# alibaba/easydist

Measured on NVIDIA H100. Metric: train_step_throughput, higher is better.
Workload: dtype bf16

## Files before the change

### easydist_b200/_lib.py

```python
import ctypes
import os
from ctypes import (POINTER, c_char_p, c_float, c_int, c_int64, c_size_t, c_uint64, c_void_p)

from . import build as _build

EDB_OK, EDB_E_INVALID, EDB_E_UNSUPPORTED, EDB_E_CUDA, EDB_E_STATE = 0, 1, 2, 3, 4

DTYPE_CODES = {"float32": 0, "bfloat16": 1, "float16": 2, "float64": 3, "int32": 4, "int64": 5}
REDOP_CODES = {"sum": 0, "max": 1, "min": 2, "avg": 3}


class EdbError(RuntimeError):

    def __init__(self, code, msg):
        super().__init__(f"libedb error {code}: {msg}")
        self.code = code


class EdbUnsupported(EdbError):
    """The kernel does not cover this shape/layout; the dispatcher may route elsewhere."""


_I64P = POINTER(c_int64)
_IP = POINTER(c_int)

SIGNATURES = {
    "edb_version": (c_int, []),
    "edb_last_error": (c_char_p, []),
    "edb_init": (c_int, [c_int, c_int, c_int, c_size_t]),
    "edb_finalize": (c_int, []),
    "edb_is_initialized": (c_int, []),
    "edb_health": (c_int, []),
    "edb_heap_info": (c_int, [POINTER(c_void_p), POINTER(c_size_t), POINTER(c_size_t)]),
    "edb_ipc_export": (c_int, [c_void_p]),
    "edb_ipc_attach": (c_int, [c_int, c_void_p]),
    "edb_attach_local": (c_int, [c_int, c_void_p]),
    "edb_group_create": (c_int, [_IP, c_int, c_int, _IP]),
    "edb_group_info": (c_int, [c_int, _IP, _IP]),
    "edb_symm_alloc": (c_int, [c_size_t, c_size_t, POINTER(c_uint64)]),
    "edb_symm_mark": (c_int, [POINTER(c_uint64)]),
    "edb_symm_reset": (c_int, [c_uint64]),
    "edb_scatter": (c_int, [c_void_p, c_void_p, _I64P, c_int, c_int, c_int, c_int, c_int, _I64P,
                            c_void_p]),
    "edb_copy": (c_int, [c_void_p, c_void_p, c_size_t, c_void_p]),
    "edb_box_copy_local": (c_int, [c_void_p, _I64P, c_void_p, _I64P, _I64P, c_int, c_int,
                                   c_void_p]),
    "edb_all_gather": (c_int, [c_int, c_uint64, c_void_p, _I64P, c_int, c_int, c_int, c_void_p]),
    "edb_reduce_scatter": (c_int, [c_int, c_void_p, c_uint64, c_void_p, _I64P, c_int, c_int, c_int,
                                   c_int, c_float, c_int, c_void_p]),
    "edb_all_reduce": (c_int, [c_int, c_void_p, c_uint64, c_uint64, c_void_p, c_int64, c_int, c_int,
                               c_void_p]),
    "edb_all_to_all": (c_int, [c_int, c_void_p, c_uint64, c_void_p, _I64P, c_int, c_int, c_int,
                               c_int, c_void_p]),
    "edb_box_exchange": (c_int, [c_int, c_void_p, _I64P, c_uint64, c_void_p, _I64P, c_int, c_int,
                                 c_int, _IP, _I64P, _I64P, _I64P, _I64P, c_void_p]),
    "edb_halo_exchange": (c_int, [c_int, c_void_p, c_uint64, c_void_p, _I64P, c_int, c_int, c_int,
                                  c_int, c_void_p]),
    "edb_symm_guard": (c_int, [c_int, c_void_p]),
    "edb_gemm_bf16": (c_int, [c_void_p, c_void_p, c_void_p, c_void_p, c_int64, c_int64, c_int64,
                              c_int64, c_int64, c_int64, c_int, c_int, c_int, c_void_p]),
    "edb_ag_gemm_bf16": (c_int, [c_int, c_void_p, c_void_p, c_void_p, c_uint64, c_uint64, c_int64,
                                 c_int64, c_int64, c_int64, c_int64, c_void_p]),
    "edb_gemm_rs_bf16": (c_int, [c_int, c_void_p, c_uint64, c_void_p, c_void_p, c_int64, c_int64,
                                 c_int64, c_int64, c_int64, c_int, c_int, c_float, c_int,
                                 c_void_p]),
    "edb_gemm_rs_push_bf16": (c_int, [c_int, c_uint64, c_uint64, c_void_p, c_void_p, c_int64, c_int64,
                                      c_int64, c_int64, c_int64, c_int, c_int, c_void_p]),
    "edb_rs_finish": (c_int, [c_int, c_int, c_void_p, c_void_p, c_void_p, _I64P, c_float, c_int,
                              c_void_p]),
    "edb_epoch_barrier": (c_int, [c_int, c_void_p]),
    "edb_all_gather_push": (c_int, [c_int, c_uint64, c_void_p, _I64P, c_int, c_int, c_int, c_void_p]),
    "edb_all_to_all_push": (c_int, [c_int, c_uint64, c_void_p, _I64P, c_int, c_int, c_int, c_int,
                                    c_void_p]),
    "edb_reduce_scatter_push": (c_int, [c_int, c_void_p, c_uint64, c_void_p, _I64P, c_int, c_int,
                                        c_int, c_int, c_float, c_int, c_void_p]),
    "edb_all_reduce_push": (c_int, [c_int, c_uint64, c_uint64, c_void_p, c_int64, c_int, c_int,
                                    c_void_p]),
    "edb_ag_gemm_epoch_bf16": (c_int, [c_int, c_void_p, c_void_p, c_void_p, c_uint64, c_uint64,
                                       c_int64, c_int64, c_int64, c_int64, c_int64, c_void_p]),
    "edb_ag_prefetch": (c_int, [c_int, c_int, c_void_p, c_void_p, _I64P, _I64P, _I64P, c_void_p]),
    "edb_gemm_pf_bf16": (c_int, [c_void_p, c_void_p, c_void_p, c_void_p, c_int64, c_int64, c_int64,
                                 c_int64, c_int64, c_int64, c_int, c_int, c_int, c_int, c_void_p,
                                 c_void_p, _I64P, _I64P, _I64P, c_void_p]),
    "edb_gemm_epi_bf16": (c_int, [c_void_p, c_void_p, c_void_p, c_void_p, c_void_p, c_int64, c_int,
                                  c_int64, c_int64, c_int64, c_int64, c_int64, c_int64, c_int, c_int,
                                  c_int, c_int, c_void_p, c_void_p, _I64P, _I64P, _I64P, c_void_p]),
    "edb_gemm_push_bf16": (c_int, [c_int, c_uint64, c_void_p, c_void_p, c_int64, c_int64, c_int64,
                                   c_int64, c_int64, c_int, c_int, c_void_p]),
    "edb_rs_finish_local": (c_int, [c_int, c_int, c_void_p, c_void_p, _I64P, c_float, c_int,
                                    c_void_p]),
    "edb_layer_norm_fwd": (c_int, [c_void_p, c_void_p, c_void_p, c_void_p, c_void_p, c_void_p,
                                   c_int64, c_int64, c_float, c_int, c_void_p]),
    "edb_layer_norm_bwd": (c_int, [c_void_p, c_void_p, c_void_p, c_void_p, c_void_p, c_void_p,
                                   c_void_p, c_void_p, c_void_p, c_int64, c_int64, c_int, c_void_p]),
    "edb_layer_norm_bwd_add": (c_int, [c_void_p, c_void_p, c_void_p, c_void_p, c_void_p, c_void_p,
                                       c_void_p, c_void_p, c_void_p, c_void_p, c_int64, c_int64,
                                       c_int, c_void_p]),
    "edb_layer_norm_bwd_workspace": (c_int, [c_int64, POINTER(c_size_t)]),
    "edb_rms_norm_fwd": (c_int, [c_void_p, c_void_p, c_void_p, c_void_p, c_int64, c_int64, c_float,
                                 c_int, c_int, c_void_p]),
    "edb_rms_norm_bwd": (c_int, [c_void_p, c_void_p, c_void_p, c_void_p, c_void_p, c_void_p, c_void_p,
                                 c_void_p, c_int64, c_int64, c_int, c_int, c_void_p]),
    "edb_rms_norm_bwd_workspace": (c_int, [c_int64, POINTER(c_size_t)]),
    "edb_swiglu_fwd": (c_int, [c_void_p, c_void_p, c_void_p, c_int64, c_int, c_void_p]),
    "edb_rope": (c_int, [c_void_p, c_void_p, c_void_p, c_void_p, c_int64, c_int64, c_int64, c_int64,
                         _I64P, _I64P, c_int64, c_int, c_int, c_void_p]),
    "edb_swiglu_bwd": (c_int, [c_void_p, c_void_p, c_void_p, c_void_p, c_void_p, c_int64, c_int,
                               c_void_p]),
    "edb_embedding_fwd": (c_int, [c_void_p, c_void_p, c_void_p, c_void_p, c_void_p, c_int64, c_int64,
                                  c_int64, c_int64, c_int64, c_int, c_int, c_void_p]),
    "edb_embedding_bwd": (c_int, [c_void_p, c_int64, c_void_p, c_int64, c_void_p, c_void_p, c_int64,
                                  c_int64, c_int64, c_int64, c_int, c_int, c_int, c_void_p]),
    "edb_embedding_bwd_workspace": (c_int, [c_int64, c_int64, POINTER(c_size_t)]),
    "edb_colsum": (c_int,[c_void_p, c_void_p, c_void_p, c_int64, c_int64, c_int64, c_int, c_void_p]),
    "edb_colsum_workspace": (c_int, [c_int64, POINTER(c_size_t)]),
    "edb_cross_entropy_fwd": (c_int, [c_void_p, c_void_p, c_void_p, c_void_p, c_void_p, c_int64,
                                      c_void_p, c_int64, c_int64, c_int64, c_int, c_int, c_void_p]),
    "edb_cross_entropy_bwd": (c_int, [c_void_p, c_int64, c_void_p, c_int64, c_void_p, c_void_p,
                                      c_void_p, c_void_p, c_int64, c_int64, c_int64, c_int, c_int,
                                      c_void_p]),
    "edb_sgd_momentum": (c_int, [c_int, c_void_p, c_void_p, c_void_p, _I64P, c_float, c_float, c_float,
                                 c_int, c_void_p]),
    "edb_sgd_momentum_scaled": (c_int, [c_int, c_void_p, c_void_p, c_void_p, _I64P, c_float, c_float,
                                        c_float, c_void_p, c_int, c_void_p]),
    "edb_grad_sumsq": (c_int, [c_int, c_void_p, _I64P, c_void_p, c_void_p, c_int, c_int, c_void_p]),
    "edb_grad_sumsq_workspace": (c_int, [c_int, _I64P, c_int, POINTER(c_size_t)]),
    "edb_multi_scale_": (c_int, [c_int, c_void_p, _I64P, c_void_p, c_int, c_void_p]),
    "edb_set_option": (c_int, [c_char_p, c_int64]),
    "edb_get_option": (c_int, [c_char_p, POINTER(c_int64)]),
    "edb_launch_count": (c_uint64, []),
}

_lib = None


def lib_path():
    return _build.LIB_PATH


def load(build_if_missing=True):
    global _lib
    if _lib is not None:
        return _lib
    path = lib_path()
    if build_if_missing and _build._nvcc() is not None and _build.needs_build():
        _build.build()
    if not os.path.exists(path):
        raise EdbError(EDB_E_STATE,
                       f"{path} is missing and cannot be built here (no nvcc); run "
                       "`python -m easydist_b200.build` where nvcc is available")
    lib = ctypes.CDLL(path, mode=ctypes.RTLD_GLOBAL)
    for name, (restype, argtypes) in SIGNATURES.items():
        fn = getattr(lib, name)
        fn.restype = restype
        fn.argtypes = argtypes
    _lib = lib
    return lib


def check(rc):
    if rc == EDB_OK:
        return
    msg = load().edb_last_error().decode("utf-8", "replace")
    if rc == EDB_E_UNSUPPORTED:
        raise EdbUnsupported(rc, msg)
    raise EdbError(rc, msg)


def i64_array(values):
    values = [int(v) for v in values]
    return (c_int64 * max(1, len(values)))(*values)


def int_array(values):
    values = [int(v) for v in values]
    return (c_int * max(1, len(values)))(*values)
```

### easydist_b200/api.py

```python
import logging
from functools import update_wrapper
from typing import Any

import os

import torch
import torch.utils._pytree as pytree

from . import lowering
from . import reshard as _default_ops
from .compile import EDCompiledFunc, GraphIO, trace_train_step
from .device_mesh import get_device_mesh

logger = logging.getLogger(__name__)

DP_MODES = ("ddp", "zero2", "zero3")
PARALLEL_EXTENTION = {}


def register_parallel_method(parallel_mode: str, compiler_func=None):

    def wrapper(fn):
        PARALLEL_EXTENTION[parallel_mode] = fn
        return fn

    return wrapper if compiler_func is None else wrapper(compiler_func)


def _dp_group(mesh):
    if "dp" in mesh.dim_names:
        d = mesh.dim_names.index("dp")
    else:
        assert mesh.ndim == 1, "data-parallel modes need a mesh dim named 'dp'"
        d = 0
    return mesh.ranks_along(d), mesh.get_coordinate()[d]


def _flat_inputs(params, buffers, named_states, args, kwargs):
    return pytree.tree_flatten((params, buffers, named_states, args, kwargs))[0]


def _single_group(gm, ops, ranks):
    want = list(ranks)
    for nd in gm.graph.nodes:
        if nd.op == "call_function" and nd.target in ops.COMM_FUNCS:
            grp = nd.args[5] if nd.target is ops.all_to_all_start else \
                (nd.args[3] if nd.target is ops.reduce_scatter_start else nd.args[2])
            if list(grp) != want:
                return False
    return True


class _ParamIO:

    def __init__(self, param_ph, param_names):
        self.param_ph, self.param_names = list(param_ph), list(param_names)


def _finish(gm, params, buffers, named_states, args, kwargs, ops, native, io=None, ranks=None,
            fuse=True, fuse_rt=None, my_index=None, auto_io=None):
    flat = _flat_inputs(params, buffers, named_states, args, kwargs)
    lowering.propagate_local_meta(gm, flat)
    info = {}
    if io is None and os.environ.get("EDB_LOCALIZE_OPT", "1" if native else "0") == "1":
        info["localized_foreach"] = lowering.localize_foreach(gm, ops, my_rank=get_device_mesh().rank)
        lowering.propagate_local_meta(gm, flat)
    auto_pf = (native or fuse_rt is not None) and fuse and auto_io is not None and ranks is not None \
        and len(ranks) > 1 and os.environ.get("EDB_EPOCH", "1") == "1" \
        and os.environ.get("EDB_AG_PREFETCH", "1") == "1"
    bucket = os.environ.get("EDB_BUCKET_COMM", "0") == "1"
    if bucket and not auto_pf:
        info["bucketed"] = lowering.bucket_small_comm(gm, ops)
        lowering.propagate_local_meta(gm, flat)
    experimental = [k for k in ("EDB_OVERLAP", "EDB_RS_LANE", "EDB_GEMM_SIDE", "EDB_DEFER_RS")
                    if os.environ.get(k, "0") == "1"]
    if experimental and native:
        if os.environ.get("EDB_ALLOW_EXPERIMENTAL", "0") != "1":
            raise RuntimeError(
                f"{experimental}: experimental multi-stream switches are gated on GPUs (kernels that "
                "spin on peer / sibling CTAs are sized for an idle GPU and are not co-residency safe "
                "next to a second stream); set EDB_ALLOW_EXPERIMENTAL=1 to try them anyway")
        logger.warning("experimental switches %s enabled (EDB_ALLOW_EXPERIMENTAL=1): not "
                       "co-residency safe, not part of the measured configuration", experimental)
    overlap = os.environ.get("EDB_OVERLAP", "0") == "1" and io is not None and ranks is not None \
        and len(ranks) > 1
    if overlap:
        info["overlap"] = lowering.overlap_schedule(gm, io, ops)
    elif (native or fuse_rt is not None) and fuse and io is not None and ranks is not None \
            and len(ranks) > 1:
        if fuse_rt is None:
            from .runtime import get_runtime
            fuse_rt = get_runtime()
        rt = fuse_rt
        rehomed, nf = lowering.fuse_collective_gemms(gm, io, rt, ranks, ops, my_index=my_index)
        info["fused"] = nf
        name_of = {ph.name: io.param_names[i] for i, ph in enumerate(io.param_ph)}
        for ph_name, buf in rehomed.items():
            pname = name_of[ph_name]
            t = params[pname]
            home = buf.tensor(t.dtype, t.shape)
            home.copy_(t)
            params[pname] = home
        lowering.propagate_local_meta(gm, _flat_inputs(params, buffers, named_states, args,
                                                       kwargs))
    elif auto_pf:
        if fuse_rt is None:
            from .runtime import get_runtime
            fuse_rt = get_runtime()
        rt = fuse_rt
        rehomed, n_pf = lowering.prefetch_param_gathers(gm, auto_io, rt, ranks, ops, my_index=my_index)
        if rehomed:
            lowering.insert_epoch_barriers(gm, ranks, ops)
            name_of = dict(zip([ph.name for ph in auto_io.param_ph], auto_io.param_names))
            for ph_name, buf in rehomed.items():
                t = params[name_of[ph_name]]
                home = buf.tensor(t.dtype, t.shape)
                home.copy_(t)
                params[name_of[ph_name]] = home
            lowering.propagate_local_meta(gm, _flat_inputs(params, buffers, named_states, args, kwargs))
        info["fused"] = {"ag_mm": 0, "ag_pf": n_pf, "mm_rs": 0}
        if bucket:
            info["bucketed"] = lowering.bucket_small_comm(gm, ops)
            lowering.propagate_local_meta(gm, _flat_inputs(params, buffers, named_states, args, kwargs))
    info["comm_nodes"] = lowering.count_nodes(gm, ops)
    info["reinplaced_updates"] = lowering.reinplace_optimizer_updates(gm)
    if native:
        from .runtime import get_runtime
        push = ranks is not None and len(ranks) > 1 and os.environ.get("EDB_EPOCH", "1") == "1" \
            and os.environ.get("EDB_PUSH_COLL", "1") == "1" and hasattr(ops, "epoch_barrier") \
            and not overlap and _single_group(gm, ops, ranks)
        info["symm_bytes"] = lowering.assign_static_buffers(gm, get_runtime(), ops, push=push)
        if push and any(nd.kwargs.get("_push") for nd in gm.graph.nodes if nd.op == "call_function"):
            lowering.ensure_end_barrier(gm, ranks, ops)
            info["push_collectives"] = True
        counts = {}
        info["gemm_nodes"] = lowering.dispatch_compute(gm, counts)
        info["rms_norm_nodes"] = counts["rms_norm"]
        info["swiglu_nodes"] = counts["swiglu"]
        info["rope_nodes"] = counts["rope"]
        info["clip_nodes"] = counts["clip"]
        info["embed_nodes"] = counts["embed"]
        if ranks is not None and len(ranks) > 1 and (push or info.get("fused")):
            try:
                rep = lowering.verify_epoch_protocol(gm, ops, len(ranks))
            except Exception as e:
                rep = {"ok": None, "problems": [f"checker failed: {e!r}"]}
            info["epoch_check"] = {"ok": rep["ok"], "problems": rep["problems"][:5],
                                   "ranges": rep.get("ranges"), "items": rep.get("items")}
            if rep["problems"]:
                logger.error("epoch-protocol check: %s", rep["problems"][:5])
                if os.environ.get("EDB_VERIFY_STRICT", "0") == "1":
                    raise RuntimeError(f"epoch-protocol check failed: {rep['problems'][:5]}")
    gm.graph.lint()
    gm.recompile()
    return info


def _compile_dp(func, parallel_mode, tracing_mode, args, kwargs, *, ops=_default_ops,
                native=True, fuse=True, bucket_numel=None, fuse_rt=None):
    mode = parallel_mode.replace("b200_", "")
    assert mode in DP_MODES, parallel_mode
    ranks, my_index = _dp_group(get_device_mesh())
    n = len(ranks)
    if bucket_numel is None:
        bucket_numel = 65536 if native else 0

    def trace_and_rewrite(a, kw, warm_up=True):
        params, buffers, named_states, gm, module, opt = trace_train_step(func, a, kw, tracing_mode,
                                                                          warm_up=warm_up)
        io = GraphIO(gm, params, buffers, named_states)
        shard_info = {}
        if n > 1:
            if mode == "ddp":
                lowering.transform_ddp(gm, io, ranks, ops, bucket_numel=bucket_numel)
            else:
                _, shard_info = lowering.transform_fsdp(gm, io, ranks, my_index,
                                                        shard_param=(mode == "zero3"), ops=ops,
                                                        bucket_numel=bucket_numel)
        return params, buffers, named_states, gm, io, shard_info

    params, buffers, named_states, gm, io, shard_info = trace_and_rewrite(args, kwargs)
    with torch.no_grad():
        params = {k: v.detach() for k, v in params.items()}
        if shard_info:
            ph_names = {ph.name: i for i, ph in enumerate(io.param_ph)}
            for ph_name, idx in ph_names.items():
                if ph_name in shard_info:
                    name = io.param_names[idx]
                    params[name] = ops.scatter_wrapper(params[name].flatten(), n, 0, my_index)
            flat_states, spec = pytree.tree_flatten(named_states)
            for i, ph in enumerate(io.state_ph):
                if ph.name in shard_info and isinstance(flat_states[i], torch.Tensor):
                    flat_states[i] = ops.scatter_wrapper(flat_states[i].detach().flatten(), n, 0,
                                                         my_index)
            named_states = pytree.tree_unflatten(flat_states, spec)
    info = _finish(gm, params, buffers, named_states, args, kwargs, ops, native, io=io,
                   ranks=ranks, fuse=fuse, fuse_rt=fuse_rt, my_index=my_index)
    info.update(mode=mode, dp_size=n)
    if native and n > 1:
        from .runtime import get_runtime
        get_runtime().host_barrier()

    def mono_compiler(compiled, a, kw):
        _, _, _, gm2, io2, _ = trace_and_rewrite(a, kw, warm_up=False)
        p, b, st = compiled.get_state()
        _finish(gm2, p, b, st, a, kw, ops, native, io=io2, ranks=ranks, fuse=False)
        return gm2

    return EDCompiledFunc(gm, params, buffers, named_states, info=info, mono_compiler=mono_compiler)


def _lower_auto(gm, plan, state_io_map, params, buffers, named_states, args, kwargs, *, ops, native,
                planner, mesh, fuse_rt=None):
    n_p, n_b = len(params), len(buffers)
    flat_states, spec = pytree.tree_flatten(named_states)
    placeholders = [n for n in gm.graph.nodes if n.op == "placeholder"]
    param_ph = placeholders[:n_p]
    buffer_ph = placeholders[n_p:n_p + n_b]
    state_ph = placeholders[n_p + n_b:n_p + n_b + len(flat_states)]
    input_phs = placeholders[n_p + n_b + len(flat_states):]
    plan = lowering._normalise_plan(plan)
    lowering.sharding_transform(gm, plan, state_io_map, ops=ops, mesh=mesh, planner=planner)
    env = gm._edb_shard_env

    def shard_local(t, ph):
        strat = env.get(ph.name)
        if not isinstance(t, torch.Tensor) or strat is None:
            return t
        coord = mesh.get_coordinate()
        for mdim, s in enumerate(strat):
            if s.is_shard():
                t = ops.scatter_wrapper(t, mesh.size(mdim), s.dim, coord[mdim])
        return t

    with torch.no_grad():
        params = {k: shard_local(v.detach(), ph) for (k, v), ph in zip(params.items(), param_ph)}
        buffers = {k: shard_local(v.detach(), ph) for (k, v), ph in zip(buffers.items(),
                                                                       buffer_ph)}
        flat_states = [shard_local(s.detach() if isinstance(s, torch.Tensor) else s, ph)
                       for s, ph in zip(flat_states, state_ph)]
        named_states = pytree.tree_unflatten(flat_states, spec)

    def input_transform(a, kw):
        flat, spec_in = pytree.tree_flatten((a, kw))
        flat = [shard_local(x.detach() if isinstance(x, torch.Tensor) else x, ph)
                for x, ph in zip(flat, input_phs)]
        return pytree.tree_unflatten(flat, spec_in)

    largs, lkwargs = input_transform(args, kwargs)
    auto_io, ranks1d, my_index = None, None, None
    if mesh.ndim == 1:
        auto_io = _ParamIO(param_ph, list(params.keys()))
        ranks1d, my_index = mesh.ranks_along(0), mesh.get_coordinate()[0]
    info = _finish(gm, params, buffers, named_states, largs, lkwargs, ops, native, auto_io=auto_io,
                   ranks=ranks1d, my_index=my_index, fuse_rt=fuse_rt)
    info.update(mode="auto", mesh=mesh.shape)
    if native:
        from .runtime import get_runtime, is_initialized
        if is_initialized():
            get_runtime().host_barrier()
    return EDCompiledFunc(gm, params, buffers, named_states, input_transform=input_transform,
                          info=info)


def _compile_auto(func, tracing_mode, args, kwargs, *, plan=None, ops=_default_ops, native=True,
                  planner="GREEDY", bundle=None):
    mesh = get_device_mesh("spmd")
    if bundle is not None:
        return compile_from_bundle(bundle, args, kwargs, ops=ops, native=native, planner=planner)
    if plan is None:
        raise NotImplementedError(
            "parallel_mode='auto' needs a sharding plan: use easydist_b200.api.register() to run "
            "behind the reference's solver, or pass plan=<plan> / bundle=<recorded graph+plan>")
    params, buffers, named_states, gm, module, opt = trace_train_step(func, args, kwargs,
                                                                      tracing_mode)
    io = GraphIO(gm, params, buffers, named_states)
    return _lower_auto(gm, plan, io.state_io_map(), params, buffers, named_states, args, kwargs,
                       ops=ops, native=native, planner=planner, mesh=mesh)


def compile_from_bundle(bundle_text, args, kwargs, *, ops=_default_ops, native=True,
                        planner="GREEDY", fuse_rt=None):
    from . import graph_io
    from .compile import find_module_and_optimizer, warm_up_optimizer
    mesh = get_device_mesh("spmd")
    module, opt = find_module_and_optimizer(args, kwargs)
    device = next(module.parameters()).device
    gm, plan, state_io, _ = graph_io.load_bundle(bundle_text, device=device.type)
    params = dict(module.named_parameters())
    buffers = dict(module.named_buffers())
    named_states = warm_up_optimizer(module, opt)
    flat = [x.detach() if isinstance(x, torch.Tensor) else None
            for x in _flat_inputs(params, buffers, named_states, args, kwargs)]
    lowering.propagate_local_meta(gm, flat)
    class _Named:
        def __init__(self, name):
            self.name = name

    io_map = {_Named(a): _Named(b) for a, b in state_io}
    return _lower_auto(gm, plan, io_map, params, buffers, named_states, args, kwargs, ops=ops,
                       native=native, planner=planner, mesh=mesh, fuse_rt=fuse_rt)


LAST_AUTO_SOURCE = [None]


def _plan_cache_key(args, kwargs, mesh):
    import hashlib
    leaves, spec = pytree.tree_flatten((args, kwargs))
    parts = [repr(spec), repr(tuple(mesh.shape))]
    for x in leaves:
        if isinstance(x, torch.Tensor):
            parts.append(f"T{tuple(x.shape)}:{x.dtype}")
        elif isinstance(x, torch.nn.Module):
            parts.append(repr(x) + "|" + ",".join(f"{n}{tuple(p.shape)}{p.dtype}"
                                                  for n, p in x.named_parameters()))
        elif isinstance(x, torch.optim.Optimizer):
            parts.append(type(x).__qualname__ + repr([{k: v for k, v in g.items() if k != "params"}
                                                      for g in x.param_groups]))
        else:
            parts.append(repr(x))
    return hashlib.sha256("|".join(parts).encode("utf-8")).hexdigest()[:32]


def input_signature(args, kwargs):
    import hashlib
    leaves, spec = pytree.tree_flatten((args, kwargs))
    parts = [repr(spec)]
    for x in leaves:
        if isinstance(x, torch.Tensor):
            parts.append(f"T{tuple(x.shape)}:{x.dtype}")
        elif isinstance(x, (torch.nn.Module, torch.optim.Optimizer)):
            parts.append(f"{type(x).__qualname__}@{id(x):x}")
        else:
            parts.append(repr(x))
    return hashlib.sha256("|".join(parts).encode("utf-8")).hexdigest()


class CompiledFuncWrapper:

    def __init__(self, func, parallel_mode="auto", tracing_mode="fake", cuda_graph=True,
                 enable_mono_graph=False, compile_only=False, compile_kwargs=None):
        update_wrapper(self, func)
        self.original_func = func
        self.compiled_func = None
        self.parallel_mode = parallel_mode
        self.tracing_mode = tracing_mode
        self.enable_cuda_graph = cuda_graph
        self.enable_mono_graph = enable_mono_graph
        self.compile_only = compile_only
        self.compile_kwargs = compile_kwargs or {}
        self.all_input_signature = []
        self.graph_list = {}
        self.cuda_graph_space = {}
        self.graph_pool = None

    def _compile(self, args, kwargs):
        mode = self.parallel_mode
        if mode == "auto":
            return _compile_auto(self.original_func, self.tracing_mode, args, kwargs,
                                 **self.compile_kwargs)
        if mode in DP_MODES:
            return _compile_dp(self.original_func, mode, self.tracing_mode, args, kwargs,
                               **self.compile_kwargs)
        if mode in PARALLEL_EXTENTION:
            return PARALLEL_EXTENTION[mode](self.original_func, mode, self.tracing_mode, args,
                                            kwargs)
        raise NotImplementedError()

    def register_input_signature(self, *args, **kwargs):
        sig = input_signature(args, kwargs)
        if sig not in self.all_input_signature:
            self.all_input_signature.append(sig)
            if self.enable_cuda_graph:
                self.cuda_graph_space[sig] = {"cuda_graph": None, "cuda_graph_input": None,
                                              "cuda_graph_output": None}
        return sig

    def _run(self, sig, args, kwargs):
        if sig not in self.graph_list:
            if not self.enable_mono_graph:
                raise RuntimeError(
                    "Input mismatch. If you are sure that different inputs do not change the graph, "
                    "you can try turning on the enable_mono_graph option.")
            self.graph_list[sig] = self.compiled_func.compile_mono_graph(*args, **kwargs)
            logger.info(f"[Compile API] compile mono graph for {sig}")
        return self.compiled_func.run_with_graph(self.graph_list[sig], *args, **kwargs)

    def __call__(self, *args: Any, **kwargs: Any) -> Any:
        sig = self.register_input_signature(*args, **kwargs)
        if self.compiled_func is None:
            self.compiled_func = self._compile(args, kwargs)
            self.graph_list[sig] = self.compiled_func.graph
        if self.compile_only:
            return self.compiled_func
        if not self.enable_cuda_graph:
            return self._run(sig, args, kwargs)
        space = self.cuda_graph_space[sig]
        flat, spec = pytree.tree_flatten([args, kwargs])
        if space["cuda_graph"] is None:
            space["cuda_graph_input"] = [torch.empty_like(x).copy_(x) if isinstance(x, torch.Tensor)
                                         else x for x in flat]
            sargs, skwargs = pytree.tree_unflatten(space["cuda_graph_input"], spec)
            s = torch.cuda.Stream()
            s.wait_stream(torch.cuda.current_stream())
            with torch.cuda.stream(s):
                space["cuda_graph_output"] = self._run(sig, sargs, skwargs)
            torch.cuda.current_stream().wait_stream(s)
            torch.cuda.synchronize()
            space["cuda_graph"] = torch.cuda.CUDAGraph()
            with torch.cuda.graph(space["cuda_graph"], self.graph_pool):
                space["cuda_graph_output"] = self._run(sig, sargs, skwargs)
            if self.graph_pool is None:
                self.graph_pool = space["cuda_graph"].pool()
        else:
            for dst, src in zip(space["cuda_graph_input"], flat):
                if isinstance(dst, torch.Tensor):
                    dst.copy_(src, non_blocking=True)
        from .compile import _check_health
        _check_health()
        space["cuda_graph"].replay()
        return space["cuda_graph_output"]


def easydist_compile(func=None, parallel_mode="auto", tracing_mode="fake", cuda_graph=True,
                     enable_mono_graph=False, use_hint=False, liveness_only_input=False,
                     max_solver_time=float("inf"), compile_only=False, **compile_kwargs):
    if parallel_mode not in ("auto",) + DP_MODES and parallel_mode not in PARALLEL_EXTENTION:
        raise NotImplementedError(
            "please use [auto, ddp, zero2, zero3] for `parallel_mode` or register your parallel "
            "extention")

    def wrap(f):
        return CompiledFuncWrapper(f, parallel_mode, tracing_mode, cuda_graph, enable_mono_graph,
                                   compile_only, compile_kwargs)

    return wrap(func) if func else wrap


def register(reference_api=None, reference_compile_auto=None, **compile_kwargs):
    import easydist.torch.api as ref_api
    import easydist.torch.compile_auto as ref_auto
    reference_api = reference_api or ref_api
    reference_compile_auto = reference_compile_auto or ref_auto
# ... 75 lines not shown
```

### easydist_b200/build.py

```python
import hashlib
import os
import shutil
import subprocess
import sys
from concurrent.futures import ThreadPoolExecutor

HERE = os.path.dirname(os.path.abspath(__file__))
ROOT = os.path.dirname(HERE)
CSRC = os.path.join(HERE, "csrc")
INCLUDE = os.path.join(ROOT, "include")
LIB_PATH = os.path.join(HERE, "libedb.so")
BUILD_DIR = os.path.join(HERE, "csrc", "_build")

HEADERS = ["edb_internal.cuh", "edb_vec.cuh"]
SOURCES = ["edb_runtime.cu", "edb_reshard.cu", "edb_ll.cu", "edb_norm.cu", "edb_rms.cu", "edb_rope.cu", "edb_embed.cu", "edb_loss.cu", "edb_optim.cu", "edb_clip.cu", "edb_gemm.cu"]

ARCH = "arch=compute_90a,code=sm_90a"

NVCC_FLAGS = [
    "-std=c++17", "-O3", "-lineinfo",
    "-gencode", ARCH,
    "-Xcompiler", "-fPIC",
    "-I", INCLUDE, "-I", CSRC,
]


def _nvcc():
    cand = shutil.which("nvcc") or "/usr/local/cuda/bin/nvcc"
    return cand if os.path.exists(cand) else None


def _digest(paths):
    h = hashlib.sha256()
    for p in sorted(paths):
        with open(p, "rb") as f:
            h.update(p.encode())
            h.update(f.read())
    h.update(" ".join(NVCC_FLAGS).encode())
    return h.hexdigest()


def sources():
    return [os.path.join(CSRC, s) for s in SOURCES if os.path.exists(os.path.join(CSRC, s))]


def needs_build():
    stamp = os.path.join(BUILD_DIR, "stamp")
    if not os.path.exists(LIB_PATH) or not os.path.exists(stamp):
        return True
    deps = sources() + [os.path.join(CSRC, h) for h in HEADERS] + [os.path.join(INCLUDE, "edb.h")]
    with open(stamp) as f:
        return f.read().strip() != _digest(deps)


def build(force=False, verbose=False):
    if not force and not needs_build():
        return LIB_PATH
    import fcntl
    os.makedirs(BUILD_DIR, exist_ok=True)
    with open(os.path.join(BUILD_DIR, ".lock"), "w") as lock:
        fcntl.flock(lock, fcntl.LOCK_EX)
        try:
            if not force and not needs_build():
                return LIB_PATH
            return _build_locked(verbose)
        finally:
            fcntl.flock(lock, fcntl.LOCK_UN)


def _build_locked(verbose):
    import tempfile
    nvcc = _nvcc()
    if nvcc is None:
        raise RuntimeError("nvcc not found: cannot build libedb.so")
    srcs = sources()
    tmp = tempfile.mkdtemp(prefix="tmp_", dir=BUILD_DIR)
    objs = [os.path.join(tmp, os.path.basename(s)[:-3] + ".o") for s in srcs]

    def compile_one(args):
        src, obj = args
        cmd = [nvcc, *NVCC_FLAGS, "-c", src, "-o", obj]
        if verbose:
            cmd.insert(1, "-Xptxas=-v")
        r = subprocess.run(cmd, capture_output=True, text=True)
        if r.returncode != 0:
            raise RuntimeError(f"nvcc failed for {src}:\n{r.stdout}\n{r.stderr}")
        return r.stderr

    with ThreadPoolExecutor(max_workers=len(srcs)) as ex:
        logs = list(ex.map(compile_one, zip(srcs, objs)))
    if verbose:
        sys.stderr.write("\n".join(logs))
    tmp_lib = os.path.join(tmp, "libedb.so")
    cmd = [nvcc, "-shared", "-gencode", ARCH, "-o", tmp_lib, *objs]
    r = subprocess.run(cmd, capture_output=True, text=True)
    if r.returncode != 0:
        raise RuntimeError(f"link failed:\n{r.stdout}\n{r.stderr}")
    deps = srcs + [os.path.join(CSRC, h) for h in HEADERS] + [os.path.join(INCLUDE, "edb.h")]
    tmp_stamp = os.path.join(tmp, "stamp")
    with open(tmp_stamp, "w") as f:
        f.write(_digest(deps))
    os.replace(tmp_lib, LIB_PATH)
    os.replace(tmp_stamp, os.path.join(BUILD_DIR, "stamp"))
    shutil.rmtree(tmp, ignore_errors=True)
    return LIB_PATH


if __name__ == "__main__":
    print(build(force="--force" in sys.argv, verbose="-v" in sys.argv))
```

### easydist_b200/csrc/edb_gemm.cu

```cuda
#include <cuda.h>
#include <cuda_bf16.h>

#include "edb_internal.cuh"

namespace edb {

constexpr int BM = 128;
constexpr int BK = 64;
constexpr int MMA_K = 16;
constexpr int kConsumerThreads = 256;
constexpr int kGemmThreads = kConsumerThreads + 32;
constexpr int kSmemABytes = BM * BK * 2;

template <int BN> struct TileCfg {
  static constexpr int kSmemBBytes = BN * BK * 2;
  static constexpr int kStageBytes = kSmemABytes + kSmemBBytes;
  static constexpr int kStages = (BN == 256) ? 4 : 6;
  static constexpr int kEpiBufBytes = BM * 64 * 2;
  static constexpr int kEpiBufs = 2;
  static constexpr int kSmemBytes =
      kStages * kStageBytes + kEpiBufs * kEpiBufBytes + 1024  + 256 ;
};


__device__ __forceinline__ uint32_t smem_u32(const void* p) {
  return static_cast<uint32_t>(__cvta_generic_to_shared(p));
}
__device__ __forceinline__ void mbar_init(uint64_t* bar, uint32_t count) {
  asm volatile("mbarrier.init.shared::cta.b64 [%0], %1;" ::"r"(smem_u32(bar)), "r"(count));
}
__device__ __forceinline__ void mbar_expect_tx(uint64_t* bar, uint32_t bytes) {
  asm volatile("mbarrier.arrive.expect_tx.shared::cta.b64 _, [%0], %1;" ::"r"(smem_u32(bar)),
               "r"(bytes)
               : "memory");
}
__device__ __forceinline__ void mbar_arrive(uint64_t* bar) {
  asm volatile("mbarrier.arrive.shared::cta.b64 _, [%0];" ::"r"(smem_u32(bar)) : "memory");
}
__device__ __forceinline__ bool mbar_try_wait(uint32_t addr, uint32_t parity) {
  uint32_t ok;
  asm volatile(
      "{\n"
      ".reg .pred p;\n"
      "mbarrier.try_wait.parity.shared::cta.b64 p, [%1], %2;\n"
      "selp.u32 %0, 1, 0, p;\n"
      "}\n"
      : "=r"(ok)
      : "r"(addr), "r"(parity)
      : "memory");
  return ok != 0;
}
__device__ __forceinline__ void mbar_wait(uint64_t* bar, uint32_t parity) {
  const uint32_t addr = smem_u32(bar);
  if (mbar_try_wait(addr, parity)) return;
  const uint64_t t0 = globaltimer_ns();
  uint32_t spins = 0;
  while (!mbar_try_wait(addr, parity)) {
    if ((++spins & 0xfff) == 0 && globaltimer_ns() - t0 > 4000000000ull) {
      asm volatile("trap;");
    }
  }
}
__device__ __forceinline__ void fence_barrier_init() {
  asm volatile("fence.mbarrier_init.release.cluster;" ::: "memory");
}
__device__ __forceinline__ void fence_proxy_async() {
  asm volatile("fence.proxy.async.shared::cta;" ::: "memory");
}
__device__ __forceinline__ void tma_load_2d(const CUtensorMap* map, uint64_t* bar, void* smem,
                                            int c0, int c1) {
  asm volatile(
      "cp.async.bulk.tensor.2d.shared::cluster.global.mbarrier::complete_tx::bytes [%0], [%1, {%3, "
      "%4}], [%2];" ::"r"(smem_u32(smem)),
      "l"(map), "r"(smem_u32(bar)), "r"(c0), "r"(c1)
      : "memory");
}
__device__ __forceinline__ void tma_store_2d(const CUtensorMap* map, const void* smem, int c0,
                                             int c1) {
  asm volatile(
      "cp.async.bulk.tensor.2d.global.shared::cta.bulk_group [%0, {%2, %3}], [%1];" ::"l"(map),
      "r"(smem_u32(smem)), "r"(c0), "r"(c1)
      : "memory");
}
__device__ __forceinline__ void tma_store_commit() {
  asm volatile("cp.async.bulk.commit_group;" ::: "memory");
}
template <int N> __device__ __forceinline__ void tma_store_wait_read() {
  asm volatile("cp.async.bulk.wait_group.read %0;" ::"n"(N) : "memory");
}
__device__ __forceinline__ void tma_store_wait_all() {
  asm volatile("cp.async.bulk.wait_group 0;" ::: "memory");
}
__device__ __forceinline__ void epi_bar_sync() {
  asm volatile("bar.sync 1, %0;" ::"n"(kConsumerThreads) : "memory");
}
__device__ __forceinline__ void prefetch_tmap(const CUtensorMap* map) {
  asm volatile("prefetch.tensormap [%0];" ::"l"(map) : "memory");
}
__device__ __forceinline__ void wgmma_fence() {
  asm volatile("wgmma.fence.sync.aligned;" ::: "memory");
}
__device__ __forceinline__ void wgmma_commit() {
  asm volatile("wgmma.commit_group.sync.aligned;" ::: "memory");
}
template <int N> __device__ __forceinline__ void wgmma_wait() {
  asm volatile("wgmma.wait_group.sync.aligned %0;" ::"n"(N) : "memory");
}

template <int TA, int TB>
__device__ __forceinline__ void wgmma_m64n128k16(float* d, uint64_t desc_a, uint64_t desc_b,
                                                  uint32_t scale_d) {
  asm volatile(
      "{\n"
      ".reg .pred p;\n"
      "setp.ne.b32 p, %66, 0;\n"
      "wgmma.mma_async.sync.aligned.m64n128k16.f32.bf16.bf16 "
      "{"
      "%0, %1, %2, %3, %4, %5, %6, %7, %8, %9, %10, %11, %12, %13, %14, %15, "
      "%16, %17, %18, %19, %20, %21, %22, %23, %24, %25, %26, %27, %28, %29, %30, %31, "
      "%32, %33, %34, %35, %36, %37, %38, %39, %40, %41, %42, %43, %44, %45, %46, %47, "
      "%48, %49, %50, %51, %52, %53, %54, %55, %56, %57, %58, %59, %60, %61, %62, %63"
      "}, %64, %65, p, 1, 1, %67, %68;\n"
      "}\n"
      : "+f"(d[0]), "+f"(d[1]), "+f"(d[2]), "+f"(d[3]), "+f"(d[4]), "+f"(d[5]), "+f"(d[6]), "+f"(d[7]),
        "+f"(d[8]), "+f"(d[9]), "+f"(d[10]), "+f"(d[11]), "+f"(d[12]), "+f"(d[13]), "+f"(d[14]), "+f"(d[15]),
        "+f"(d[16]), "+f"(d[17]), "+f"(d[18]), "+f"(d[19]), "+f"(d[20]), "+f"(d[21]), "+f"(d[22]), "+f"(d[23]),
        "+f"(d[24]), "+f"(d[25]), "+f"(d[26]), "+f"(d[27]), "+f"(d[28]), "+f"(d[29]), "+f"(d[30]), "+f"(d[31]),
        "+f"(d[32]), "+f"(d[33]), "+f"(d[34]), "+f"(d[35]), "+f"(d[36]), "+f"(d[37]), "+f"(d[38]), "+f"(d[39]),
        "+f"(d[40]), "+f"(d[41]), "+f"(d[42]), "+f"(d[43]), "+f"(d[44]), "+f"(d[45]), "+f"(d[46]), "+f"(d[47]),
        "+f"(d[48]), "+f"(d[49]), "+f"(d[50]), "+f"(d[51]), "+f"(d[52]), "+f"(d[53]), "+f"(d[54]), "+f"(d[55]),
        "+f"(d[56]), "+f"(d[57]), "+f"(d[58]), "+f"(d[59]), "+f"(d[60]), "+f"(d[61]), "+f"(d[62]), "+f"(d[63])
      : "l"(desc_a), "l"(desc_b), "r"(scale_d), "n"(TA), "n"(TB));
}

template <int TA, int TB>
__device__ __forceinline__ void wgmma_m64n256k16(float* d, uint64_t desc_a, uint64_t desc_b,
                                                  uint32_t scale_d) {
  asm volatile(
      "{\n"
      ".reg .pred p;\n"
      "setp.ne.b32 p, %130, 0;\n"
      "wgmma.mma_async.sync.aligned.m64n256k16.f32.bf16.bf16 "
      "{"
      "%0, %1, %2, %3, %4, %5, %6, %7, %8, %9, %10, %11, %12, %13, %14, %15, "
      "%16, %17, %18, %19, %20, %21, %22, %23, %24, %25, %26, %27, %28, %29, %30, %31, "
      "%32, %33, %34, %35, %36, %37, %38, %39, %40, %41, %42, %43, %44, %45, %46, %47, "
      "%48, %49, %50, %51, %52, %53, %54, %55, %56, %57, %58, %59, %60, %61, %62, %63, "
      "%64, %65, %66, %67, %68, %69, %70, %71, %72, %73, %74, %75, %76, %77, %78, %79, "
      "%80, %81, %82, %83, %84, %85, %86, %87, %88, %89, %90, %91, %92, %93, %94, %95, "
      "%96, %97, %98, %99, %100, %101, %102, %103, %104, %105, %106, %107, %108, %109, %110, %111, "
      "%112, %113, %114, %115, %116, %117, %118, %119, %120, %121, %122, %123, %124, %125, %126, %127"
      "}, %128, %129, p, 1, 1, %131, %132;\n"
      "}\n"
      : "+f"(d[0]), "+f"(d[1]), "+f"(d[2]), "+f"(d[3]), "+f"(d[4]), "+f"(d[5]), "+f"(d[6]), "+f"(d[7]),
        "+f"(d[8]), "+f"(d[9]), "+f"(d[10]), "+f"(d[11]), "+f"(d[12]), "+f"(d[13]), "+f"(d[14]), "+f"(d[15]),
        "+f"(d[16]), "+f"(d[17]), "+f"(d[18]), "+f"(d[19]), "+f"(d[20]), "+f"(d[21]), "+f"(d[22]), "+f"(d[23]),
        "+f"(d[24]), "+f"(d[25]), "+f"(d[26]), "+f"(d[27]), "+f"(d[28]), "+f"(d[29]), "+f"(d[30]), "+f"(d[31]),
        "+f"(d[32]), "+f"(d[33]), "+f"(d[34]), "+f"(d[35]), "+f"(d[36]), "+f"(d[37]), "+f"(d[38]), "+f"(d[39]),
        "+f"(d[40]), "+f"(d[41]), "+f"(d[42]), "+f"(d[43]), "+f"(d[44]), "+f"(d[45]), "+f"(d[46]), "+f"(d[47]),
        "+f"(d[48]), "+f"(d[49]), "+f"(d[50]), "+f"(d[51]), "+f"(d[52]), "+f"(d[53]), "+f"(d[54]), "+f"(d[55]),
        "+f"(d[56]), "+f"(d[57]), "+f"(d[58]), "+f"(d[59]), "+f"(d[60]), "+f"(d[61]), "+f"(d[62]), "+f"(d[63]),
        "+f"(d[64]), "+f"(d[65]), "+f"(d[66]), "+f"(d[67]), "+f"(d[68]), "+f"(d[69]), "+f"(d[70]), "+f"(d[71]),
        "+f"(d[72]), "+f"(d[73]), "+f"(d[74]), "+f"(d[75]), "+f"(d[76]), "+f"(d[77]), "+f"(d[78]), "+f"(d[79]),
        "+f"(d[80]), "+f"(d[81]), "+f"(d[82]), "+f"(d[83]), "+f"(d[84]), "+f"(d[85]), "+f"(d[86]), "+f"(d[87]),
        "+f"(d[88]), "+f"(d[89]), "+f"(d[90]), "+f"(d[91]), "+f"(d[92]), "+f"(d[93]), "+f"(d[94]), "+f"(d[95]),
        "+f"(d[96]), "+f"(d[97]), "+f"(d[98]), "+f"(d[99]), "+f"(d[100]), "+f"(d[101]), "+f"(d[102]), "+f"(d[103]),
        "+f"(d[104]), "+f"(d[105]), "+f"(d[106]), "+f"(d[107]), "+f"(d[108]), "+f"(d[109]), "+f"(d[110]), "+f"(d[111]),
        "+f"(d[112]), "+f"(d[113]), "+f"(d[114]), "+f"(d[115]), "+f"(d[116]), "+f"(d[117]), "+f"(d[118]), "+f"(d[119]),
        "+f"(d[120]), "+f"(d[121]), "+f"(d[122]), "+f"(d[123]), "+f"(d[124]), "+f"(d[125]), "+f"(d[126]), "+f"(d[127])
      : "l"(desc_a), "l"(desc_b), "r"(scale_d), "n"(TA), "n"(TB));
}


__device__ __forceinline__ uint64_t make_smem_desc(uint32_t smem_addr, uint32_t lbo_bytes,
                                                   uint32_t sbo_bytes) {
  uint64_t d = 0;
  d |= (uint64_t)((smem_addr >> 4) & 0x3fff);
  d |= (uint64_t)((lbo_bytes >> 4) & 0x3fff) << 16;
  d |= (uint64_t)((sbo_bytes >> 4) & 0x3fff) << 32;
  d |= (uint64_t)1 << 62;
  return d;
}

struct GemmParams {
  __nv_bfloat16* C;
  const __nv_bfloat16* bias;
  int64_t ldc;
  int M, N, K;
  int m_tiles, n_tiles;
  int splits, kb_per_split;
  float* partial;
  int64_t ldp;
  int push_n, push_mtc, m_rot;
  int push_sync;
  const __nv_bfloat16* aux;
  int64_t ld_aux;
  int epi_op;
};
enum { EPI_NONE = 0, EPI_ADD = 1, EPI_GELU_BWD = 2 };

__device__ __forceinline__ float gelu_tanh_grad(float x) {
  const float kBeta = 0.7978845608028654f;
  const float kKappa = 0.044715f;
  const float x_sq = x * x;
  const float inner = kBeta * (x + kKappa * x_sq * x);
  const float au = fabsf(inner);
  float e;
  asm("ex2.approx.ftz.f32 %0, %1;" : "=f"(e) : "f"(-2.885390081777927f * au));
  float r;
  asm("rcp.approx.ftz.f32 %0, %1;" : "=f"(r) : "f"(1.0f + e));
  const float t = copysignf((1.0f - e) * r, inner);
  const float tanh_d = 4.0f * e * r * r;
  const float left = 0.5f * x, right = 1.0f + t;
  const float left_d = 0.5f * right;
  const float inner_d = kBeta * (1.0f + 3.0f * kKappa * x_sq);
  return left_d + left * tanh_d * inner_d;
}

enum { MODE_PLAIN = 0, MODE_AG = 1, MODE_RS = 2 };
constexpr int kMaxPfItems = 4;
constexpr int kPfSlots = 12, kPfDepth = 8;
constexpr int F_TILECNT = 96;

struct FusedArgs {
  FlagCtx f;
  int n_comm;
  const char* shard_src[kMaxGroup];
  char* full_dst;
  int64_t shard_bytes;
  int ag_rows;
  int ag_first_tile;
  char* recv_base;
  int64_t chunk_bytes;
  void* rs_dst;
  float rs_scale;
  int rs_out_dtype;
  int tiles_per_chunk;
  int rs_defer;
  uint64_t* rs_state;
  int epoch;
  int pf_ctas, pf_items, pf_n;
  const char* pf_heap[kMaxGroup];
  char* pf_local;
  uint64_t pf_src[kMaxPfItems], pf_dst[kMaxPfItems];
  int64_t pf_bytes[kMaxPfItems], pf_stride[kMaxPfItems];
  int64_t pf_sstride[kMaxPfItems];
  int pf_inplace[kMaxPfItems];
};
constexpr int F_PUSHED = F_CHUNK + 8;

struct CMaps {
  CUtensorMap m[kMaxGroup];
};

template <int MODE>
__device__ __forceinline__ void tile_coords(int t, const GemmParams& p, const FusedArgs& fa,
                                            int& m_blk, int& n_blk, int& chunk) {
  if (MODE == MODE_AG) {
    const int ni = t / p.m_tiles;
    n_blk = (fa.ag_first_tile + ni) % p.n_tiles;
    m_blk = t - ni * p.m_tiles;
    chunk = -1;
  } else if (MODE == MODE_RS) {
    const int mtc = p.m_tiles / fa.f.n;
    const int tpc = mtc * p.n_tiles;
    const int ci = t / tpc, w = t - ci * tpc;
    chunk = (fa.f.me + 1 + ci) % fa.f.n;
    m_blk = chunk * mtc + w % mtc;
    n_blk = w / mtc;
  } else {
    chunk = 0;
    m_blk = (t % p.m_tiles + p.m_rot) % p.m_tiles;
    n_blk = t / p.m_tiles;
  }
}

__device__ __forceinline__ void bulk_load(void* smem, const void* gsrc, uint32_t bytes,
                                          uint64_t* bar) {
  asm volatile(
      "cp.async.bulk.shared::cluster.global.mbarrier::complete_tx::bytes [%0], [%1], %2, [%3];" ::
          "r"(smem_u32(smem)),
      "l"(gsrc), "r"(bytes), "r"(smem_u32(bar))
      : "memory");
}
__device__ __forceinline__ void bulk_store(void* gdst, const void* smem, uint32_t bytes) {
  asm volatile("cp.async.bulk.global.shared::cta.bulk_group [%0], [%1], %2;" ::"l"(gdst),
               "r"(smem_u32(smem)), "r"(bytes)
               : "memory");
}
__device__ __forceinline__ void fence_proxy_async_all() {
  asm volatile("fence.proxy.async;" ::: "memory");
}
__device__ __forceinline__ void spin_wait_gpu(const uint64_t* flag, uint64_t target) {
  if (ld_acquire_gpu(flag) >= target) return;
  const uint64_t t0 = globaltimer_ns();
  uint32_t spins = 0;
  while (ld_acquire_gpu(flag) < target) {
    __nanosleep(32);
    if ((++spins & 0xfff) == 0 && globaltimer_ns() - t0 > 4000000000ull) asm volatile("trap;");
  }
}

__device__ __forceinline__ void pf_role(const FusedArgs& fa, uint8_t* smem, int idx, int nctas) {
  constexpr int S = kPfSlots, D = kPfDepth, SLOT = 16384;
  uint64_t* full = reinterpret_cast<uint64_t*>(smem + S * SLOT);
  if (threadIdx.x == 0) {
    for (int s = 0; s < S; ++s) mbar_init(&full[s], 1);
    fence_barrier_init();
  }
  __syncthreads();
  if (threadIdx.x != 0) return;
  uint32_t n_load = 0, n_store = 0;
  struct Cur { int it, k; int64_t blk; };
  auto advance = [&](Cur& c) {
    while (c.it < fa.pf_items) {
      const int64_t nblk = (fa.pf_bytes[c.it] + SLOT - 1) / SLOT;
      const int members = fa.pf_inplace[c.it] ? fa.pf_n - 1 : fa.pf_n;
      if (c.k < members && c.blk < nblk) return true;
      if (c.k < members) c.blk -= nblk;
      if (++c.k >= members) {
        c.k = 0;
        ++c.it;
      }
    }
    return false;
  };
  Cur ld = {0, 0, (int64_t)idx}, stc = {0, 0, (int64_t)idx};
  bool more = advance(ld);
  int inflight = 0;
  while (more || inflight > 0) {
    if (more && inflight < D) {
      const uint32_t slot = n_load % S;
      if (n_load >= (uint32_t)S) tma_store_wait_read<S - D - 1>();
      const int p = (fa.f.me + 1 + ld.k) % fa.pf_n;
      const int64_t off = ld.blk * SLOT;
      const int64_t left = fa.pf_bytes[ld.it] - off;
      const uint32_t bytes = (uint32_t)(left < SLOT ? left : SLOT);
      mbar_expect_tx(&full[slot], bytes);
      bulk_load(smem + slot * SLOT,
                fa.pf_heap[p] + fa.pf_src[ld.it] + (int64_t)p * fa.pf_sstride[ld.it] + off, bytes,
                &full[slot]);
      ++n_load;
      ++inflight;
      ld.blk += nctas;
      more = advance(ld);
      continue;
    }
    advance(stc);
    const uint32_t slot = n_store % S;
    mbar_wait(&full[slot], (n_store / S) & 1);
    const int p = (fa.f.me + 1 + stc.k) % fa.pf_n;
    const int64_t off = stc.blk * SLOT;
    const int64_t left = fa.pf_bytes[stc.it] - off;
    const uint32_t bytes = (uint32_t)(left < SLOT ? left : SLOT);
    bulk_store(fa.pf_local + fa.pf_dst[stc.it] + (int64_t)p * fa.pf_stride[stc.it] + off,
               smem + slot * SLOT, bytes);
    tma_store_commit();
    ++n_store;
    --inflight;
    stc.blk += nctas;
  }
  tma_store_wait_all();
}

__global__ void __launch_bounds__(32, 1) k_ag_prefetch(const __grid_constant__ FusedArgs fa) {
  extern __shared__ uint8_t pf_smem_raw[];
  uint8_t* smem = reinterpret_cast<uint8_t*>((reinterpret_cast<uintptr_t>(pf_smem_raw) + 1023) &
                                             ~static_cast<uintptr_t>(1023));
  pf_role(fa, smem, (int)blockIdx.x, (int)gridDim.x);
}

__device__ __forceinline__ void ag_comm_role_epoch(const FusedArgs& fa, uint8_t* smem, int comm_idx,
                                                   uint64_t q) {
  constexpr int S = 8, D = 5, SLOT = 16384, kLag = 2;
  uint64_t* full = reinterpret_cast<uint64_t*>(smem + S * SLOT);
  const FlagCtx& f = fa.f;
  if (threadIdx.x == 0) {
    for (int s = 0; s < S; ++s) mbar_init(&full[s], 1);
    fence_barrier_init();
  }
  __syncthreads();
  if (threadIdx.x != 0) return;
  const int64_t per = ((fa.shard_bytes + fa.n_comm - 1) / fa.n_comm + SLOT - 1) / SLOT * SLOT;
  const int64_t lo = (int64_t)comm_idx * per;
  const int64_t hi = lo + per < fa.shard_bytes ? lo + per : fa.shard_bytes;
  const int nblk = hi > lo ? (int)((hi - lo + SLOT - 1) / SLOT) : 0;
  const int total = nblk * f.n;
  auto announce = [&](int k) {
    const int c = (f.me + k) % f.n;
    const unsigned long long prev =
        atomicAdd(reinterpret_cast<unsigned long long*>(f.local + F_AGTILE + c), 1ULL);
    if (prev == (unsigned long long)fa.n_comm - 1) {
      f.local[F_AGTILE + c] = 0;
      __threadfence();
      st_release_gpu(f.local + F_AGCHUNK + c, q);
    }
  };
  if (nblk == 0) {
    for (int k = 0; k < f.n; ++k) announce(k);
  } else {
    uint32_t n_load = 0, n_store = 0;
    int next_announce = 0;
    for (int g = 0; g < total + D; ++g) {
      if (g < total) {
        const int k = g / nblk, i = g - k * nblk;
        const int c = (f.me + k) % f.n;
        const uint32_t slot = n_load % S;
        if (n_load >= (uint32_t)S) tma_store_wait_read<S - D - 1>();
        const int64_t left = hi - lo - (int64_t)i * SLOT;
        const uint32_t bytes = (uint32_t)(left < SLOT ? left : SLOT);
        mbar_expect_tx(&full[slot], bytes);
        bulk_load(smem + slot * SLOT, fa.shard_src[c] + lo + (int64_t)i * SLOT, bytes, &full[slot]);
        ++n_load;
      }
      if (g >= D) {
        const int j = g - D;
        const int k = j / nblk, i = j - k * nblk;
        const int c = (f.me + k) % f.n;
        const uint32_t slot = n_store % S;
        mbar_wait(&full[slot], (n_store / S) & 1);
        const int64_t left = hi - lo - (int64_t)i * SLOT;
        const uint32_t bytes = (uint32_t)(left < SLOT ? left : SLOT);
        bulk_store(fa.full_dst + (int64_t)c * fa.shard_bytes + lo + (int64_t)i * SLOT,
                   smem + slot * SLOT, bytes);
        tma_store_commit();
        ++n_store;
        if ((int)n_store - kLag >= (next_announce + 1) * nblk) {
          asm volatile("cp.async.bulk.wait_group %0;" ::"n"(kLag) : "memory");
          fence_proxy_async_all();
          __threadfence();
          while ((int)n_store - kLag >= (next_announce + 1) * nblk) announce(next_announce++);
        }
      }
    }
    tma_store_wait_all();
    fence_proxy_async_all();
    __threadfence();
    while (next_announce < f.n) announce(next_announce++);
  }
  const unsigned long long prev =
      atomicAdd(reinterpret_cast<unsigned long long*>(f.local + F_AGDONE), 1ULL);
  if (prev == (unsigned long long)fa.n_comm - 1) {
    f.local[F_AGDONE] = 0;
    while (ld_acquire_gpu(f.local + F_AGCNT) < (uint64_t)gridDim.x) __nanosleep(64);
    f.local[F_AGCNT] = 0;
    st_release_gpu(f.local + F_AGSEQ, q);
  }
}

__device__ __forceinline__ void ag_comm_role(const FusedArgs& fa, uint8_t* smem, int comm_idx,
                                             uint64_t q) {
  constexpr int S = 8, D = 4, SLOT = 16384;
  uint64_t* full = reinterpret_cast<uint64_t*>(smem + S * SLOT);
  const FlagCtx& f = fa.f;
  if (threadIdx.x == 0) {
    for (int s = 0; s < S; ++s) mbar_init(&full[s], 1);
    fence_barrier_init();
  }
  __syncthreads();
  if (threadIdx.x != 0) return;
  const int w_chunk = F_CHUNK, w_tile = F_TILECNT;
  if (comm_idx == 0) {
    __threadfence_system();
    for (int pidx = 0; pidx < f.n; ++pidx)
      if (pidx != f.me) st_release_sys(f.peer[pidx] + F_READY + f.me, q);
  }
  uint32_t n_load = 0, n_store = 0;
  const int64_t per = ((fa.shard_bytes + fa.n_comm - 1) / fa.n_comm + SLOT - 1) / SLOT * SLOT;
  const int64_t lo = (int64_t)comm_idx * per;
  const int64_t hi = lo + per < fa.shard_bytes ? lo + per : fa.shard_bytes;
  const int64_t nblk = hi > lo ? (hi - lo + SLOT - 1) / SLOT : 0;
  for (int k = 0; k < f.n; ++k) {
    const int c = (f.me + k) % f.n;
    if (c != f.me) spin_wait_sys(f.local + F_READY + c, q, f.timeout_ns, f.local + F_ERR);
    const char* src = fa.shard_src[c] + lo;
    char* dst = fa.full_dst + (int64_t)c * fa.shard_bytes + lo;
    for (int64_t i = 0; i < nblk + D; ++i) {
      if (i < nblk) {
        const uint32_t slot = n_load % S;
        if (n_load >= (uint32_t)S) tma_store_wait_read<S - D - 1>();
        const int64_t left = hi - lo - i * SLOT;
        const uint32_t bytes = (uint32_t)(left < SLOT ? left : SLOT);
        mbar_expect_tx(&full[slot], bytes);
        bulk_load(smem + slot * SLOT, src + i * SLOT, bytes, &full[slot]);
// ... 118 lines not shown

template <int BN, bool A_KMAJOR, bool B_KMAJOR, int MODE>
__global__ void __launch_bounds__(kGemmThreads, 1)
    k_gemm_bf16(const __grid_constant__ CUtensorMap tmap_a, const __grid_constant__ CUtensorMap tmap_b,
                const __grid_constant__ CUtensorMap tmap_c, const GemmParams p,
                const __grid_constant__ FusedArgs fa, const __grid_constant__ CMaps cm) {
  using Cfg = TileCfg<BN>;
  constexpr int kStages = Cfg::kStages;
  extern __shared__ uint8_t smem_raw[];
  uint8_t* smem = reinterpret_cast<uint8_t*>((reinterpret_cast<uintptr_t>(smem_raw) + 1023) &
                                             ~static_cast<uintptr_t>(1023));
  __shared__ uint64_t s_q;
  __shared__ int s_last;
  uint64_t q = 0;
  const int n_gemm_ctas = (MODE == MODE_AG) ? (int)gridDim.x - fa.n_comm
                                             : (MODE == MODE_PLAIN ? (int)gridDim.x - fa.pf_ctas : (int)gridDim.x);

  if (MODE == MODE_RS) {
    if (fa.rs_defer) {
      if (threadIdx.x == 0) s_q = ld_relaxed_gpu(fa.f.local + F_SEQ) + 1;
      if ((int)threadIdx.x < fa.f.n && (int)threadIdx.x != fa.f.me) {
        const uint64_t prev = ld_relaxed_gpu(fa.rs_state + 1);
        if (prev) spin_wait_sys(fa.f.local + F_DONE + threadIdx.x, prev, fa.f.timeout_ns, fa.f.local + F_ERR);
      }
      __syncthreads();
      q = s_q;
    } else {
      q = begin_op(fa.f, &s_q);
    }
  } else if (MODE == MODE_AG) {
    if (threadIdx.x == 0) {
      s_q = ld_relaxed_gpu(fa.f.local + (fa.epoch ? F_AGSEQ : F_SEQ)) + 1;
      atomicAdd(reinterpret_cast<unsigned long long*>(fa.f.local + (fa.epoch ? F_AGCNT : F_CNT_C)), 1ULL);
    }
    __syncthreads();
    q = s_q;
    if ((int)blockIdx.x < fa.n_comm) {
      if (fa.epoch) ag_comm_role_epoch(fa, smem, (int)blockIdx.x, q);
      else ag_comm_role(fa, smem, (int)blockIdx.x, q);
      return;
    }
  }
  if (MODE == MODE_PLAIN && fa.pf_ctas > 0 && (int)blockIdx.x < fa.pf_ctas) {
    pf_role(fa, smem, (int)blockIdx.x, fa.pf_ctas);
    return;
  }
  const int cta = (MODE == MODE_AG) ? (int)blockIdx.x - fa.n_comm
                                    : (MODE == MODE_PLAIN ? (int)blockIdx.x - fa.pf_ctas : (int)blockIdx.x);

  uint8_t* smem_a = smem;
  uint8_t* smem_b = smem + kStages * kSmemABytes;
  uint8_t* smem_epi = smem + kStages * Cfg::kStageBytes;
  uint64_t* bars = reinterpret_cast<uint64_t*>(smem_epi + Cfg::kEpiBufs * Cfg::kEpiBufBytes);
  uint64_t* full_bar = bars;
  uint64_t* empty_bar = bars + kStages;

  const int warp = threadIdx.x >> 5;
  const int lane = threadIdx.x & 31;
  const int k_blocks = (p.K + BK - 1) / BK;
  const int num_tiles = p.m_tiles * p.n_tiles;
  const int num_units = (MODE == MODE_PLAIN) ? num_tiles * p.splits : num_tiles;

  if (threadIdx.x == 0) {
    for (int s = 0; s < kStages; ++s) {
      mbar_init(&full_bar[s], 1);
      mbar_init(&empty_bar[s], 2);
    }
    fence_barrier_init();
  }
  __syncthreads();

  if (warp == kConsumerThreads / 32) {
    if (lane == 0) {
      prefetch_tmap(&tmap_a);
      prefetch_tmap(&tmap_b);
      int stage = 0;
      uint32_t phase = 0;
      int ready_chunk = -1;
      for (int u = cta; u < num_units; u += n_gemm_ctas) {
        const int t = (MODE == MODE_PLAIN) ? u % num_tiles : u;
        int kb0 = 0, kb1 = k_blocks;
        if (MODE == MODE_PLAIN && p.splits > 1) {
          kb0 = (u / num_tiles) * p.kb_per_split;
          kb1 = kb0 + p.kb_per_split < k_blocks ? kb0 + p.kb_per_split : k_blocks;
        }
        int m_blk, n_blk, chunk;
        tile_coords<MODE>(t, p, fa, m_blk, n_blk, chunk);
        const CUtensorMap* bmap = &tmap_b;
        int b_row = n_blk * BN;
        if (MODE == MODE_AG) {
          const int c_lo = (n_blk * BN) / fa.ag_rows, c_hi = (n_blk * BN + BN - 1) / fa.ag_rows;
          if (c_lo == fa.f.me && c_hi == fa.f.me) {
            bmap = &cm.m[0];
            b_row = n_blk * BN - fa.f.me * fa.ag_rows;
          } else if (n_blk != ready_chunk) {
            for (int c = c_lo; c <= c_hi; ++c)
              spin_wait_gpu(fa.f.local + (fa.epoch ? F_AGCHUNK : F_CHUNK) + c, q);
            fence_proxy_async_all();
            ready_chunk = n_blk;
          }
        }
        for (int kb = kb0; kb < kb1; ++kb) {
          mbar_wait(&empty_bar[stage], phase ^ 1);
          uint8_t* sa = smem_a + stage * kSmemABytes;
          uint8_t* sb = smem_b + stage * Cfg::kSmemBBytes;
          mbar_expect_tx(&full_bar[stage], Cfg::kStageBytes);
          if (A_KMAJOR) {
            tma_load_2d(&tmap_a, &full_bar[stage], sa, kb * BK, m_blk * BM);
          } else {
#pragma unroll
            for (int h = 0; h < BM / 64; ++h)
              tma_load_2d(&tmap_a, &full_bar[stage], sa + h * (64 * BK * 2), m_blk * BM + h * 64,
                          kb * BK);
          }
          if (B_KMAJOR) {
            tma_load_2d(bmap, &full_bar[stage], sb, kb * BK, b_row);
          } else {
#pragma unroll
            for (int h = 0; h < BN / 64; ++h)
              tma_load_2d(bmap, &full_bar[stage], sb + h * (64 * BK * 2), b_row + h * 64, kb * BK);
          }
          if (++stage == kStages) {
            stage = 0;
            phase ^= 1;
          }
        }
      }
    }
  } else {
    const int wg = warp >> 2;
    const int tid = threadIdx.x & 127;
    const int frag_row = 16 * (tid >> 5) + ((tid & 31) >> 2);
    const int frag_col = 2 * (tid & 3);
    const int row0 = wg * 64 + frag_row;
    const bool issuer = (threadIdx.x == 0);
    if (issuer) prefetch_tmap(&tmap_c);
    float acc[BN / 2];
    int stage = 0;
    uint32_t phase = 0;
    int ebuf = 0;
    for (int u = cta; u < num_units; u += n_gemm_ctas) {
      const int t = (MODE == MODE_PLAIN) ? u % num_tiles : u;
      int kb0 = 0, kb1 = k_blocks;
      if (MODE == MODE_PLAIN && p.splits > 1) {
        kb0 = (u / num_tiles) * p.kb_per_split;
        kb1 = kb0 + p.kb_per_split < k_blocks ? kb0 + p.kb_per_split : k_blocks;
      }
      int m_blk, n_blk, chunk;
      tile_coords<MODE>(t, p, fa, m_blk, n_blk, chunk);

      int prev = -1;
      for (int kb = kb0; kb < kb1; ++kb) {
        mbar_wait(&full_bar[stage], phase);
        wgmma_fence();
        mma_k_block<BN, A_KMAJOR, B_KMAJOR>(acc, smem_u32(smem_a + stage * kSmemABytes) + wg * (64 * BK * 2),
                                            smem_u32(smem_b + stage * Cfg::kSmemBBytes), kb == kb0);
        wgmma_commit();
        wgmma_wait<1>();
        if (prev >= 0 && tid == 0) mbar_arrive(&empty_bar[prev]);
        prev = stage;
        if (++stage == kStages) {
          stage = 0;
          phase ^= 1;
        }
      }
      wgmma_wait<0>();
      if (prev >= 0 && tid == 0) mbar_arrive(&empty_bar[prev]);

      if (MODE == MODE_PLAIN && p.splits > 1) {
#pragma unroll
        for (int h = 0; h < 2; ++h) {
          const int64_t r = (int64_t)m_blk * BM + row0 + 8 * h;
          if (r >= p.M) continue;
          float* prow = p.partial + ((int64_t)(u / num_tiles) * p.M + r) * p.ldp;
#pragma unroll
          for (int j = 0; j < BN / 8; ++j) {
            const int col = n_blk * BN + 8 * j + frag_col;
            if (col < p.ldp)
              *reinterpret_cast<float2*>(prow + col) = make_float2(acc[4 * j + 2 * h], acc[4 * j + 2 * h + 1]);
          }
        }
        continue;
      }
      const CUtensorMap* cmap = &tmap_c;
      int c_row = m_blk * BM;
      if (MODE == MODE_RS) {
        cmap = &cm.m[chunk];
        c_row = (m_blk - chunk * (p.m_tiles / fa.f.n)) * BM;
      }
      if (MODE == MODE_PLAIN && p.push_n > 0) {
        const int owner = m_blk / p.push_mtc;
        cmap = &cm.m[owner];
        c_row = (m_blk - owner * p.push_mtc) * BM;
      }
      const bool has_aux = (MODE == MODE_PLAIN && p.epi_op != EPI_NONE);
#pragma unroll
      for (int c0 = 0; c0 < BN; c0 += 64) {
        float* v = acc + c0 / 2;
        if (p.bias != nullptr) {
#pragma unroll
          for (int j = 0; j < 8; ++j) {
            const int col = n_blk * BN + c0 + 8 * j + frag_col;
            if (col < p.N) {
              const float2 f = __bfloat1622float2(*reinterpret_cast<const __nv_bfloat162*>(p.bias + col));
#pragma unroll
              for (int h = 0; h < 2; ++h) {
                v[4 * j + 2 * h] += f.x;
                v[4 * j + 2 * h + 1] += f.y;
              }
            }
          }
        }
        if (has_aux) {
#pragma unroll
          for (int h = 0; h < 2; ++h) {
            const int64_t r = (int64_t)m_blk * BM + row0 + 8 * h;
            const __nv_bfloat16* arow = p.aux + r * p.ld_aux;
#pragma unroll
            for (int j = 0; j < 8; ++j) {
              const int col = n_blk * BN + c0 + 8 * j + frag_col;
              float2 f = make_float2(0.f, 0.f);
              if (r < p.M && col < p.N)
                f = __bfloat1622float2(*reinterpret_cast<const __nv_bfloat162*>(arow + col));
              float x0 = v[4 * j + 2 * h], x1 = v[4 * j + 2 * h + 1];
              if (p.epi_op == EPI_ADD) {
                x0 += f.x;
                x1 += f.y;
              } else {
                x0 = __bfloat162float(__float2bfloat16_rn(x0)) * gelu_tanh_grad(f.x);
                x1 = __bfloat162float(__float2bfloat16_rn(x1)) * gelu_tanh_grad(f.y);
              }
              v[4 * j + 2 * h] = x0;
              v[4 * j + 2 * h + 1] = x1;
            }
          }
        }
        if (issuer) tma_store_wait_read<Cfg::kEpiBufs - 1>();
        epi_bar_sync();
        uint8_t* buf = smem_epi + ebuf * Cfg::kEpiBufBytes;
#pragma unroll
        for (int h = 0; h < 2; ++h) {
          const int row = row0 + 8 * h;
          uint8_t* rowp = buf + row * 128 + frag_col * 2;
#pragma unroll
          for (int j = 0; j < 8; ++j) {
            __nv_bfloat162 o = __floats2bfloat162_rn(v[4 * j + 2 * h], v[4 * j + 2 * h + 1]);
            *reinterpret_cast<__nv_bfloat162*>(rowp + ((j ^ (row & 7)) << 4)) = o;
          }
        }
        fence_proxy_async();
        epi_bar_sync();
        if (issuer) {
          tma_store_2d(cmap, buf, n_blk * BN + c0, c_row);
          tma_store_commit();
        }
        ebuf ^= 1;
      }
      if (MODE == MODE_RS && issuer) {
        tma_store_wait_all();
        fence_proxy_async_all();
        __threadfence_system();
        const unsigned long long prev_cnt = atomicAdd(
            reinterpret_cast<unsigned long long*>(fa.f.local + F_TILECNT + chunk), 1ULL);
        if (prev_cnt == (unsigned long long)fa.tiles_per_chunk - 1) {
          fa.f.local[F_TILECNT + chunk] = 0;
          __threadfence_system();
          st_release_sys(fa.f.peer[chunk] + (fa.rs_defer ? F_PUSHED : F_CHUNK) + fa.f.me, q);
        }
      }
    }
    if (issuer) {
      if (MODE == MODE_PLAIN && p.push_n > 0 && p.push_sync == 0) {
        tma_store_wait_read<0>();
      } else {
        tma_store_wait_all();
        if (MODE == MODE_PLAIN && p.push_n > 0 && p.push_sync >= 2) {
          fence_proxy_async_all();
          __threadfence_system();
        }
      }
    }
  }

  if (MODE == MODE_RS) {
    __syncthreads();
    if (fa.rs_defer) {
      if (blockIdx.x == 0 && threadIdx.x == 0) fa.rs_state[0] = q;
    } else {
      if (threadIdx.x < fa.f.n)
        spin_wait_sys(fa.f.local + F_CHUNK + threadIdx.x, q, fa.f.timeout_ns, fa.f.local + F_ERR);
      __syncthreads();
      const uint64_t tid = (uint64_t)blockIdx.x * blockDim.x + threadIdx.x;
      const uint64_t nthr = (uint64_t)gridDim.x * blockDim.x;
      if (fa.rs_out_dtype == EDB_F32) rs_tail_reduce<float>(fa, tid, nthr);
      else rs_tail_reduce<__nv_bfloat16>(fa, tid, nthr);
    }
    finish_op(fa.f, q, &s_last, gridDim.x);
  }
}

constexpr int kGemm2Threads = 384;
constexpr int kGemm2EpiBufBytes = 64 * 64 * 2;

template <int R> __device__ __forceinline__ void setmaxnreg_dec() {
  asm volatile("setmaxnreg.dec.sync.aligned.u32 %0;" ::"n"(R));
}
template <int R> __device__ __forceinline__ void setmaxnreg_inc() {
  asm volatile("setmaxnreg.inc.sync.aligned.u32 %0;" ::"n"(R));
}
__device__ __forceinline__ void wg_bar_sync(int wg) {
  if (wg == 0) asm volatile("bar.sync 1, 128;" ::: "memory");
  else asm volatile("bar.sync 2, 128;" ::: "memory");
}
__device__ __forceinline__ bool mbar_wait_ok(uint64_t* bar, uint32_t parity) {
  const uint32_t addr = smem_u32(bar);
  if (mbar_try_wait(addr, parity)) return true;
  const uint64_t t0 = globaltimer_ns();
  uint32_t spins = 0;
  while (!mbar_try_wait(addr, parity)) {
    if ((++spins & 0xfff) == 0 && globaltimer_ns() - t0 > 4000000000ull) return false;
  }
  return true;
}

template <bool A_KMAJOR, bool B_KMAJOR>
__global__ void __launch_bounds__(kGemm2Threads, 1)
    k_gemm2_bf16(const __grid_constant__ CUtensorMap tmap_a, const __grid_constant__ CUtensorMap tmap_b,
                 const __grid_constant__ CUtensorMap tmap_c, const GemmParams p) {
  constexpr int BN = 256;
  using Cfg = TileCfg<BN>;
  constexpr int kStages = Cfg::kStages;
  extern __shared__ uint8_t smem_raw[];
  uint8_t* smem = reinterpret_cast<uint8_t*>((reinterpret_cast<uintptr_t>(smem_raw) + 1023) &
                                             ~static_cast<uintptr_t>(1023));
  uint8_t* smem_a = smem;
  uint8_t* smem_b = smem + kStages * kSmemABytes;
  uint8_t* smem_epi = smem + kStages * Cfg::kStageBytes;
  uint64_t* full_bar = reinterpret_cast<uint64_t*>(smem_epi + Cfg::kEpiBufs * Cfg::kEpiBufBytes);
  uint64_t* empty_bar = full_bar + kStages;

  const int wgi = threadIdx.x >> 7;
  const int k_blocks = (p.K + BK - 1) / BK;
  const int mt = p.m_tiles;
  const int num_units = mt * p.n_tiles;

  if (threadIdx.x == 0) {
    for (int s = 0; s < kStages; ++s) {
      mbar_init(&full_bar[s], 1);
      mbar_init(&empty_bar[s], 2);
    }
    fence_barrier_init();
  }
  __syncthreads();

  bool ok = true;
  if (wgi == 0) {
    setmaxnreg_dec<40>();
    if (threadIdx.x == 0) {
      prefetch_tmap(&tmap_a);
      prefetch_tmap(&tmap_b);
      int stage = 0;
      uint32_t phase = 0;
      for (int u = blockIdx.x; ok && u < num_units; u += gridDim.x) {
        const int m_blk = u % mt, n_blk = u / mt;
        for (int kb = 0; kb < k_blocks; ++kb) {
          if (!(ok = mbar_wait_ok(&empty_bar[stage], phase ^ 1))) break;
          uint8_t* sa = smem_a + stage * kSmemABytes;
          uint8_t* sb = smem_b + stage * Cfg::kSmemBBytes;
          mbar_expect_tx(&full_bar[stage], Cfg::kStageBytes);
          if (A_KMAJOR) {
            tma_load_2d(&tmap_a, &full_bar[stage], sa, kb * BK, m_blk * BM);
          } else {
#pragma unroll
            for (int h = 0; h < BM / 64; ++h)
              tma_load_2d(&tmap_a, &full_bar[stage], sa + h * (64 * BK * 2), m_blk * BM + h * 64,
                          kb * BK);
          }
          if (B_KMAJOR) {
            tma_load_2d(&tmap_b, &full_bar[stage], sb, kb * BK, n_blk * BN);
          } else {
#pragma unroll
            for (int h = 0; h < BN / 64; ++h)
              tma_load_2d(&tmap_b, &full_bar[stage], sb + h * (64 * BK * 2), n_blk * BN + h * 64,
                          kb * BK);
          }
          if (++stage == kStages) {
            stage = 0;
            phase ^= 1;
          }
        }
      }
    }
  } else {
    setmaxnreg_inc<232>();
    const int wg = wgi - 1;
    const int tid = threadIdx.x & 127;
    const int frag_row = 16 * (tid >> 5) + ((tid & 31) >> 2);
    const int frag_col = 2 * (tid & 3);
    const int row0 = wg * 64 + frag_row;
    const bool issuer = (tid == 0);
    uint8_t* epi = smem_epi + wg * (2 * kGemm2EpiBufBytes);
    if (issuer) prefetch_tmap(&tmap_c);
    const int epi_op = p.epi_op;
    float acc[BN / 2];
    int stage = 0;
    uint32_t phase = 0;
    int ebuf = 0;
    for (int u = blockIdx.x; u < num_units; u += gridDim.x) {
      const int m_blk = u % mt, n_blk = u / mt;
      int prev = -1;
      for (int kb = 0; kb < k_blocks; ++kb) {
        if (!(ok = mbar_wait_ok(&full_bar[stage], phase))) break;
        wgmma_fence();
        mma_k_block<BN, A_KMAJOR, B_KMAJOR>(acc, smem_u32(smem_a + stage * kSmemABytes) + wg * (64 * BK * 2),
                                            smem_u32(smem_b + stage * Cfg::kSmemBBytes), kb == 0);
        wgmma_commit();
        wgmma_wait<1>();
        if (prev >= 0 && tid == 0) mbar_arrive(&empty_bar[prev]);
        prev = stage;
        if (++stage == kStages) {
          stage = 0;
          phase ^= 1;
        }
      }
      wgmma_wait<0>();
      if (!ok) break;
      if (prev >= 0 && tid == 0) mbar_arrive(&empty_bar[prev]);

#pragma unroll
      for (int c0 = 0; c0 < BN; c0 += 64) {
        float* v = acc + c0 / 2;
        if (p.bias != nullptr) {
#pragma unroll
          for (int j = 0; j < 8; ++j) {
            const int col = n_blk * BN + c0 + 8 * j + frag_col;
            if (col < p.N) {
              const float2 f = __bfloat1622float2(*reinterpret_cast<const __nv_bfloat162*>(p.bias + col));
#pragma unroll
              for (int h = 0; h < 2; ++h) {
                v[4 * j + 2 * h] += f.x;
                v[4 * j + 2 * h + 1] += f.y;
              }
            }
          }
        }
        if (epi_op != EPI_NONE) {
#pragma unroll
          for (int h = 0; h < 2; ++h) {
            const int64_t r = (int64_t)m_blk * BM + row0 + 8 * h;
            const __nv_bfloat16* arow = p.aux + r * p.ld_aux;
#pragma unroll
            for (int j = 0; j < 8; ++j) {
              const int col = n_blk * BN + c0 + 8 * j + frag_col;
              float2 f = make_float2(0.f, 0.f);
              if (r < p.M && col < p.N)
                f = __bfloat1622float2(*reinterpret_cast<const __nv_bfloat162*>(arow + col));
              float x0 = v[4 * j + 2 * h], x1 = v[4 * j + 2 * h + 1];
              if (epi_op == EPI_ADD) {
                x0 += f.x;
                x1 += f.y;
              } else {
                x0 = __bfloat162float(__float2bfloat16_rn(x0)) * gelu_tanh_grad(f.x);
                x1 = __bfloat162float(__float2bfloat16_rn(x1)) * gelu_tanh_grad(f.y);
              }
              v[4 * j + 2 * h] = x0;
              v[4 * j + 2 * h + 1] = x1;
            }
          }
        }
        if (issuer) tma_store_wait_read<1>();
        wg_bar_sync(wg);
        uint8_t* buf = epi + ebuf * kGemm2EpiBufBytes;
#pragma unroll
        for (int h = 0; h < 2; ++h) {
          const int row = frag_row + 8 * h;
          uint8_t* rowp = buf + row * 128 + frag_col * 2;
#pragma unroll
          for (int j = 0; j < 8; ++j) {
            __nv_bfloat162 o = __floats2bfloat162_rn(v[4 * j + 2 * h], v[4 * j + 2 * h + 1]);
            *reinterpret_cast<__nv_bfloat162*>(rowp + ((j ^ (row & 7)) << 4)) = o;
          }
        }
        fence_proxy_async();
        wg_bar_sync(wg);
        if (issuer) {
          tma_store_2d(&tmap_c, buf, n_blk * BN + c0, m_blk * BM + wg * 64);
          tma_store_commit();
        }
        ebuf ^= 1;
      }
    }
    if (issuer) tma_store_wait_all();
  }
  if (!ok) asm volatile("trap;");
}

constexpr int kRsMaxItems = 160;
constexpr int kRsFinishThreads = 256;
constexpr int64_t kRsFinishChunkVecs = 4096;

struct RsFinishItem {
  const char* recv;
  void* dst;
  int64_t chunk_bytes;
  uint64_t* state;
};
struct RsFinishDesc {
  FlagCtx f;
  int local_only;
  int n_items;
  float scale;
  int out_dtype;
  int first_unit[kRsMaxItems + 1];
  RsFinishItem it[kRsMaxItems];
};

template <int NSRC>
__global__ void __launch_bounds__(kRsFinishThreads, 4)
    k_rs_finish(const __grid_constant__ RsFinishDesc d) {
  __shared__ uint64_t s_q;
  __shared__ unsigned long long s_need;
  __shared__ int s_last;
  if (threadIdx.x == 0) {
    s_q = ld_relaxed_gpu(d.f.local + F_SEQ) + 1;
    s_need = 0;
  }
  __syncthreads();
  if (!d.local_only) {
    unsigned long long need = 0;
    for (int i = threadIdx.x; i < d.n_items; i += blockDim.x) {
      const unsigned long long e = ld_relaxed_gpu(d.it[i].state);
      need = e > need ? e : need;
    }
    if (need) atomicMax(&s_need, need);
    __syncthreads();
    if ((int)threadIdx.x < d.f.n)
      spin_wait_sys(d.f.local + F_PUSHED + threadIdx.x, s_need, d.f.timeout_ns, d.f.local + F_ERR);
    __syncthreads();
  }
  const uint64_t q = s_q;
  const int total_units = d.first_unit[d.n_items];
  const int n = NSRC > 0 ? NSRC : d.f.n;
  constexpr int MAXS = NSRC > 0 ? NSRC : kMaxGroup;
  constexpr int U = NSRC > 0 ? (8 / NSRC > 0 ? 8 / NSRC : 1) : 1;
  for (int u = blockIdx.x; u < total_units; u += gridDim.x) {
    int lo = 0, hi = d.n_items;
    while (hi - lo > 1) {
      const int mid = (lo + hi) >> 1;
      if (d.first_unit[mid] <= u) lo = mid;
      else hi = mid;
    }
    const char* recv = d.it[lo].recv;
    void* dst = d.it[lo].dst;
    const int64_t chunk_bytes = d.it[lo].chunk_bytes;
    const int64_t nvec = chunk_bytes / 16;
    const int64_t v0 = (int64_t)(u - d.first_unit[lo]) * kRsFinishChunkVecs;
    const int64_t v1 = v0 + kRsFinishChunkVecs < nvec ? v0 + kRsFinishChunkVecs : nvec;
    for (int64_t i0 = v0 + threadIdx.x; i0 < v1; i0 += U * kRsFinishThreads) {
      uint4 raw[U][MAXS];
#pragma unroll
      for (int uu = 0; uu < U; ++uu) {
        const int64_t i = i0 + uu * kRsFinishThreads;
        if (i < v1) {
#pragma unroll
          for (int sidx = 0; sidx < MAXS; ++sidx)
            if (sidx < n)
              raw[uu][sidx] = __ldcs(reinterpret_cast<const uint4*>(recv + (int64_t)sidx * chunk_bytes + i * 16));
        }
      }
#pragma unroll
      for (int uu = 0; uu < U; ++uu) {
        const int64_t i = i0 + uu * kRsFinishThreads;
        if (i >= v1) break;
        float acc[8];
#pragma unroll
        for (int sidx = 0; sidx < MAXS; ++sidx) {
          if (sidx < n) {
            const __nv_bfloat162* h = reinterpret_cast<const __nv_bfloat162*>(&raw[uu][sidx]);
#pragma unroll
            for (int e = 0; e < 4; ++e) {
              const float2 v = __bfloat1622float2(h[e]);
              if (sidx == 0) {
                acc[2 * e] = v.x;
                acc[2 * e + 1] = v.y;
              } else {
                acc[2 * e] += v.x;
                acc[2 * e + 1] += v.y;
              }
            }
          }
        }
#pragma unroll
        for (int e = 0; e < 8; ++e) acc[e] *= d.scale;
        if (d.out_dtype == EDB_F32) rs_store<float>(static_cast<float*>(dst), i, acc);
        else rs_store<__nv_bfloat16>(static_cast<__nv_bfloat16*>(dst), i, acc);
      }
    }
  }
  if (d.local_only) return;
  if (blockIdx.x == 0)
    for (int i = threadIdx.x; i < d.n_items; i += blockDim.x) d.it[i].state[1] = q;
  finish_op(d.f, q, &s_last, gridDim.x);
}

struct PushDst {
  int n;
  int64_t rows_per, row_rot;
  __nv_bfloat16* base[kMaxGroup];
};

__global__ void __launch_bounds__(256)
    k_splitk_reduce(__nv_bfloat16* __restrict__ C, int64_t ldc, const float* __restrict__ partial,
// ... 721 lines not shown
```

### easydist_b200/lowering.py

```python
import operator
import os
from typing import Dict

import torch
import torch.utils._pytree as pytree
from torch.fx.node import Node

from . import metair as M
from . import planners
from . import reshard as _default_ops
from .device_mesh import get_device_mesh

aten = torch.ops.aten

CREATE_ATEN_OP = [
    aten.empty.memory_format, aten.zeros.default, aten.ones.default, aten.scalar_tensor.default,
    aten.arange.default, aten.arange.start, aten.full.default,
]



def local_shape(global_shape, mesh, placements):
    shape = list(global_shape)
    coord = mesh.get_coordinate()
# ... 1458 lines not shown
               for nd in skip1 + skip2 for a in pytree.tree_flatten((nd.args, nd.kwargs))[0]):
            continue
        if mul.kwargs or set(add1.kwargs) - {"alpha"} or set(add2.kwargs) - {"alpha"}:
            continue
        if mul.users or add1.users or add2.users or len(mul.args) != 2:
            continue
        bufs, mu = mul.args
        if not isinstance(mu, (int, float)) or len(add1.args) != 2 or len(add2.args) != 2:
            continue
        if list(add1.args[0]) != list(bufs) or list(add2.args[1]) != list(bufs):
            continue
        grads, params = add1.args[1], add2.args[0]
        if not (len(grads) == len(bufs) == len(params)):
            continue
        if set(params) & set(bufs) or set(grads) & set(bufs) or set(grads) & set(params):
            continue
        ga, nlr = add1.kwargs.get("alpha", 1), add2.kwargs.get("alpha", 1)
        if not isinstance(ga, (int, float)) or not isinstance(nlr, (int, float)):
            continue
        with graph.inserting_before(add2):
            graph.call_function(optim.sgd_momentum_, (list(params), list(grads), list(bufs), mu, ga, nlr))
        for d in (add2, add1, mul):
            graph.erase_node(d)
        n += 1
    if n:
        gm.recompile()
    return n


_ALIAS_OPS = (aten.t.default, aten.view.default, aten._unsafe_view.default, aten.transpose.int,
              aten.permute.default, aten.alias.default, aten.detach.default, aten.slice.Tensor,
              aten.select.int, aten.flatten.using_ints, aten.reshape.default, aten.expand.default,
              aten.unsqueeze.default, aten.squeeze.dim, aten.as_strided.default)
_VIEW_ONLY = (aten.t.default, aten.view.default, aten._unsafe_view.default, aten.transpose.int,
              aten.permute.default, aten.alias.default, aten.detach.default, aten.unsqueeze.default,
              aten.squeeze.dim)


def _memory_readers(x, through=_ALIAS_OPS):
    root = x
    while _call(root, *through):
        root = root.args[0]
    readers, frontier, seen = [], [root], {root}
    while frontier:
        nd = frontier.pop()
        for u in nd.users:
            if u in seen:
                continue
            seen.add(u)
            if _call(u, *through) and u.args[0] is nd:
                frontier.append(u)
            else:
                readers.append(u)
    return readers


def _fold_clip_scale(gm, clamp):
    from . import clip, optim
    graph = gm.graph
    dt = _val(clamp).dtype if _val(clamp) is not None else None
    muls = [u for u in clamp.users if _call(u, aten.mul_.Tensor) and len(u.args) == 2
            and u.args[1] is clamp and u.args[0] is not clamp and not u.kwargs
            and _val(u.args[0]) is not None and _val(u.args[0]).dtype == dt]
    if not muls or len({m.args[0] for m in muls}) != len(muls):
        return 0
    pos = {nd: i for i, nd in enumerate(graph.nodes)}
    muls.sort(key=lambda m: pos[m])
    group = set(muls)
    users = {u for m in muls for u in m.users}
    sgd = next(iter(users)) if len(users) == 1 else None
    if _call(sgd, optim.sgd_momentum_) and "grad_scale" not in sgd.kwargs \
            and all(len(m.users) == 1 for m in muls) and set(sgd.args[1]) == group \
            and len(sgd.args[1]) == len(muls) \
            and not any(pos[r] > pos[m] and r not in group
                        for m in muls for r in _memory_readers(m.args[0])):
        args = list(sgd.args)
        args[1] = [m.args[0] for m in args[1]]
        sgd.args = tuple(args)
        sgd.kwargs = dict(sgd.kwargs, grad_scale=clamp)
        for m in muls:
            graph.erase_node(m)
        return len(muls)
    first = pos[muls[0]]
    for m in muls:
        if any(first < pos[r] < pos[m] and r not in group for r in _memory_readers(m.args[0])):
            return 0
    with graph.inserting_before(muls[0]):
        graph.call_function(clip.scale_, ([m.args[0] for m in muls], clamp))
    for m in muls:
        m.replace_all_uses_with(m.args[0])
        graph.erase_node(m)
    return len(muls)


def fuse_grad_clip(gm):
    from . import clip
    graph = gm.graph
    n_norm = n_scale = 0
    for ch in _match_clip(gm):
        norms, stack = ch["norms"], ch["stack"]
        dts = {_val(nd).dtype for nd in norms if _val(nd) is not None}
        if len(dts) != 1 or any(_val(nd.args[0]) is None or _val(nd.args[0]).dtype not in dts
                                for nd in norms):
            continue
        with graph.inserting_before(stack):
            gn = graph.call_function(clip.grad_norms, ([nd.args[0] for nd in norms],))
        gn.meta = dict(stack.meta)
        stack.replace_all_uses_with(gn)
        graph.erase_node(stack)
        for nd in norms:
            graph.erase_node(nd)
        n_norm += len(norms)
    for total in [nd for nd in graph.nodes if _is_norm2(nd)]:
        coef = _clip_coef(total)
        if coef is not None:
            n_scale += _fold_clip_scale(gm, coef[0])
    if n_norm or n_scale:
        graph.lint()
        gm.recompile()
    return n_norm, n_scale


def _embedding_pair(add):
    pair = _bin(add, aten.add.Tensor)
    if pair is None or not all(_call(e, aten.embedding.default) and _only_user(e) is add for e in pair):
        return None
    vals = [(_val(e.args[0]), _val(e.args[1])) for e in pair]
    if _val(add) is None or any(w is None or i is None for w, i in vals) or vals[0][0].dtype != vals[1][0].dtype:
        return None
    for tok, pos in ((0, 1), (1, 0)):
        (w, idx), (p, ps) = vals[tok], vals[pos]
        if ps.dim() == 1 and idx.dim() >= 1 and idx.shape[-1] == ps.shape[0] \
                and tuple(_val(add).shape) == tuple(idx.shape) + (w.shape[1],):
            return pair[tok], pair[pos]
    return None


def _tied_lm_gradient(bwd):
    from . import gemm
    add = _only_user(bwd)
    x = _other(_bin(add, aten.add.Tensor), bwd)
    root = x
    while _call(root, *_VIEW_ONLY):
        root = root.args[0]
    if not _call(root, gemm.mm) or root.kwargs.get("_side") or _memory_readers(x) != [add]:
        return None
    xv, bv, av = _val(x), _val(bwd), _val(add)
    if xv is None or bv is None or av is None or xv.dim() != 2 or xv.stride(1) != 1 \
            or tuple(xv.shape) != tuple(bv.shape) or tuple(av.shape) != tuple(xv.shape) \
            or not xv.dtype == bv.dtype == av.dtype:
        return None
    return add, x


def fuse_embedding(gm):
    from . import embed
    graph = gm.graph
    n_fwd = n_bwd = 0
    for nd in [nd for nd in graph.nodes if _call(nd, aten.add.Tensor)]:
        m = _embedding_pair(nd)
        if m is not None:
            tok, pos = m
            with graph.inserting_before(nd):
                new = graph.call_function(embed.embedding_fwd, (*tok.args[:2], *pos.args[:2]))
            new.meta = dict(nd.meta)
            nd.replace_all_uses_with(new)
            _erase_dead(graph, [nd, tok, pos])
            n_fwd += 1
    for nd in list(graph.nodes):
        if _call(nd, aten.embedding.default):
            nd.target, nd.args, nd.kwargs = embed.embedding_fwd, tuple(nd.args[:2]), {}
            n_fwd += 1
        elif _call(nd, aten.embedding_dense_backward.default) and len(nd.args) == 5 \
                and not nd.kwargs and nd.args[4] is False:
            dy, idx, V, pad, _ = nd.args
            tied = _tied_lm_gradient(nd)
            if tied is not None:
                add, x = tied
                with graph.inserting_before(add):
                    new = graph.call_function(embed.embedding_bwd_acc_, (x, dy, idx, pad))
                new.meta = dict(add.meta)
                add.replace_all_uses_with(new)
                _erase_dead(graph, [add, nd])
            else:
                nd.target, nd.args = embed.embedding_bwd, (dy, idx, V, pad)
            n_bwd += 1
    if n_fwd or n_bwd:
        graph.lint()
        gm.recompile()
    return n_fwd, n_bwd


def parallel_wgrad_gemms(gm):
    from . import gemm
    graph = gm.graph
    nodes = list(graph.nodes)
    order = {n: i for i, n in enumerate(nodes)}
    moved = 0
    for node in reversed(nodes):
        if node.op != "call_function" or node.target is not gemm.mm or node.kwargs:
            continue
        consumers = _memory_readers(node, _VIEW_ONLY)
        if not consumers:
            continue
        first = min(consumers, key=lambda u: order[u])
        between = nodes[order[node] + 1:order[first]]
        if not any(b.op == "call_function" and b.target in (gemm.mm, gemm.addmm)
                   and not b.kwargs.get("_side") for b in between):
            continue
        node.kwargs = {"_side": 1}
        with graph.inserting_before(first):
            graph.call_function(gemm.join, args=(node,))
        moved += 1
    if moved:
        graph.lint()
        gm.recompile()
    return moved


def fuse_gemm_epilogues(gm):
    from . import gemm, norm
    graph = gm.graph
    n = 0
    bf16 = torch.bfloat16

    def gemm_behind(nd):
        chain = []
        while _call(nd, aten.view.default, aten._unsafe_view.default) and len(nd.users) == 1:
            chain.append(nd)
            nd = nd.args[0]
        if _call(nd, gemm.mm, gemm.addmm) and len(nd.users) == 1 and not nd.kwargs.get("_side"):
            return nd, chain
        return None, chain

    def fuse(node, g, chain, target, operand, *extra):
        gv, ov, nv = _val(g), _val(operand), _val(node)
        with graph.inserting_before(g):
            op2d = operand if ov.dim() == 2 else graph.call_function(
                aten.view.default, args=(operand, list(gv.shape)))
            a, b = g.args[-2:]
            fused = graph.call_function(target, args=(a, b, op2d, *extra),
                                        kwargs={k: v for k, v in g.kwargs.items() if k == "_pf"})
            fused.meta = dict(g.meta)
            out = fused
            if nv.dim() != 2:
                out = graph.call_function(aten.view.default, args=(fused, list(nv.shape)))
                out.meta = dict(node.meta)
        node.replace_all_uses_with(out)
        _erase_dead(graph, [node, *chain, g])

    for node in list(graph.nodes):
        if node.op != "call_function":
            continue
        if node.target == aten.add.Tensor and len(node.args) == 2 and not node.kwargs:
            for gi, oi in ((1, 0), (0, 1)):
                g, chain = gemm_behind(node.args[gi])
                other = node.args[oi]
                gv, ov, nv = _val(g), _val(other), _val(node)
                if gv is None or ov is None or nv is None:
                    continue
                if ov.dtype != bf16 or gv.dtype != bf16 or gv.shape[1] % 8 or \
                        tuple(ov.shape) != tuple(nv.shape) or ov.numel() != gv.numel():
                    continue
                if not ov.is_contiguous():
                    continue
                order = {nd: i for i, nd in enumerate(graph.nodes)}
                if order[other] > order[g]:
                    continue
                fuse(node, g, chain, gemm.mm_add, other, g.args[0] if g.target is gemm.addmm else None)
                n += 1
                break
        elif node.target == aten.gelu_backward.default and node.kwargs.get("approximate") == "tanh":
            g, chain = gemm_behind(node.args[0])
            pre = node.args[1]
            gv, pv, nv = _val(g), _val(pre), _val(node)
            if g is None or g.target is not gemm.mm or gv is None or pv is None or nv is None:
                continue
            if pv.dtype != bf16 or gv.dtype != bf16 or gv.shape[1] % 8 or pv.numel() != gv.numel() \
                    or not pv.is_contiguous():
                continue
            order = {nd: i for i, nd in enumerate(graph.nodes)}
            if order[pre] > order[g]:
                continue
            fuse(node, g, chain, gemm.mm_gelu_bwd, pre)
            n += 1
    n += _fold_accumulation(graph, norm.native_layer_norm_backward)
    if n:
        graph.lint()
        gm.recompile()
    return n


def _reshape_views_of(node):
    frontier = [node]
    while frontier:
        nd = frontier.pop()
        for u in nd.users:
            if _call(u, *_ALIAS_OPS) and u.args[0] is nd:
                if u.target in (aten.view.default, aten._unsafe_view.default):
                    u.target = aten.reshape.default
                frontier.append(u)


def dispatch_compute(gm, counts=None):
    from . import gemm, norm
    native_ln = os.environ.get("EDB_NATIVE_LN", "1") == "1"
    counts = {} if counts is None else counts
    n = 0
    if os.environ.get("EDB_NATIVE_CE", "1") == "1":
        n += fuse_cross_entropy(gm)
    if os.environ.get("EDB_NATIVE_OPT", "1") == "1":
        n += fuse_optimizer_updates(gm)
    counts["rms_norm"] = fuse_rms_norm(gm) if os.environ.get("EDB_NATIVE_RMS", "1") == "1" else (0, 0)
    counts["swiglu"] = fuse_swiglu(gm) if os.environ.get("EDB_NATIVE_SWIGLU", "1") == "1" else (0, 0)
    counts["rope"] = fuse_rope(gm) if os.environ.get("EDB_NATIVE_ROPE", "1") == "1" else (0, 0)
    counts["clip"] = fuse_grad_clip(gm) if os.environ.get("EDB_NATIVE_CLIP", "1") == "1" else (0, 0)
    n += sum(counts["rms_norm"]) + sum(counts["swiglu"]) + sum(counts["rope"]) + sum(counts["clip"])
    for node in gm.graph.nodes:
        if node.op != "call_function":
            continue
        val = _val(node)
        if native_ln and node.target == aten.native_layer_norm.default:
            node.target = norm.native_layer_norm
            n += 1
        elif native_ln and node.target == aten.native_layer_norm_backward.default:
            node.target = norm.native_layer_norm_backward
            n += 1
        elif native_ln and node.target == aten.sum.dim_IntList:
            node.target = norm.sum_dim_intlist
            n += 1
        elif val is None or val.dtype != torch.bfloat16:
            continue
        elif node.target == aten.mm.default:
            node.target = gemm.mm
            if "edb_pf" in node.meta:
                node.kwargs = {"_pf": node.meta["edb_pf"]}
            if val.dim() == 2 and val.shape[1] % 8:
                _reshape_views_of(node)
            n += 1
        elif node.target == aten.addmm.default and not node.kwargs:
            node.target = gemm.addmm
            if "edb_pf" in node.meta:
                node.kwargs = {"_pf": node.meta["edb_pf"]}
            n += 1
    gm.recompile()
    counts["embed"] = fuse_embedding(gm) if os.environ.get("EDB_NATIVE_EMBED", "1") == "1" else (0, 0)
    n += sum(counts["embed"])
    if os.environ.get("EDB_GEMM_SIDE", "0") == "1":
        n += parallel_wgrad_gemms(gm)
    if os.environ.get("EDB_FUSE_EPILOGUE", "1") == "1":
        n += fuse_gemm_epilogues(gm)
    return n


def prefetch_param_gathers(gm, io, rt, ranks, ops=_default_ops, my_index=None):
    import os
    from collections import deque
    graph = gm.graph
    n = len(ranks)
    order = {nd: i for i, nd in enumerate(graph.nodes)}
    uses = {}
    dim1_ok = os.environ.get("EDB_AG_PREFETCH_DIM1", "1") == "1"
    for ag_s in [x for x in graph.nodes if x.op == "call_function" and x.target is ops.all_gather_start]:
        ph, n_t = ag_s.args[0], 0
        while isinstance(ph, Node) and ph.op == "call_function" and ph.target == aten.t.default and \
                isinstance(ph.args[0], Node):
            ph, n_t = ph.args[0], n_t + 1
        transposed = bool(n_t % 2)
        if not (isinstance(ph, Node) and ph.op == "placeholder" and ph in io.param_ph):
            continue
        val = ph.meta.get("val")
        if not isinstance(val, torch.Tensor) or (val.numel() * val.element_size()) % 16 or val.numel() == 0:
            continue
        if n_t and val.dim() != 2:
            continue
        d = ag_s.args[1]
        if not isinstance(d, int):
            continue
        d = d + val.dim() if d < 0 else d
        wdim = 1 - d if transposed else d
        if wdim == 1 and not (val.dim() == 2 and dim1_ok):
            continue
        if wdim not in (0, 1) or list(ag_s.args[2]) != list(ranks) \
                or ag_s.kwargs or len(ag_s.users) != 1 or not val.is_contiguous():
            continue
        ag_e = next(iter(ag_s.users))
        if ag_e.target is not ops.all_gather_end:
            continue
        uses.setdefault(ph, []).append((ag_s, ag_e, transposed, wdim))
    uses = {ph: lst for ph, lst in uses.items() if len({u[3] for u in lst}) == 1}
    if not uses:
        return {}, 0
    rehomed, bufs = {}, {}
    for ph in uses:
        nbytes = _nbytes(ph.meta["val"])
        full = rt.alloc(nbytes * n, align=1024)
        if my_index is None:
            shard = rt.alloc(nbytes, align=1024)
        else:
            shard = full.sub(int(my_index) * nbytes, nbytes)
        rehomed[ph.name] = shard
        bufs[ph] = (shard, full, nbytes)
    gathered_nodes = {}
    for ph, lst in uses.items():
        shard, full, nbytes = bufs[ph]
        pv = ph.meta["val"]
        for ag_s, ag_e, transposed, wdim in lst:
            with graph.inserting_before(ag_s):
                g = graph.call_function(ops.gathered, args=(ph, list(ranks)),
                                        kwargs={"_buf": (shard.offset, full.offset)})
                res = g
                if wdim == 1:
                    r_, c_ = pv.shape
                    res = graph.call_function(aten.view.default, args=(g, [n, r_, c_]))
                    res = graph.call_function(aten.permute.default, args=(res, [1, 0, 2]))
                    res = graph.call_function(aten.reshape.default, args=(res, [r_, n * c_]))
                elif pv.dim() > 1:
                    res = graph.call_function(aten.view.default,
                                              args=(g, [n * pv.shape[0]] + list(pv.shape[1:])))
                if transposed:
                    res = graph.call_function(aten.t.default, args=(res,))
            res.meta = dict(ag_e.meta)
            ag_e.replace_all_uses_with(res)
            graph.erase_node(ag_e)
            graph.erase_node(ag_s)
            gathered_nodes.setdefault(ph, []).append(g)
    for nd in reversed(list(graph.nodes)):
        if nd.op == "call_function" and nd.target == aten.t.default and not nd.users:
            graph.erase_node(nd)
    order = {nd: i for i, nd in enumerate(graph.nodes)}
    first_use = {ph: min(order[g] for g in gathered_nodes[ph]) for ph in uses}
    carriers = []
    for nd in graph.nodes:
        if nd.op != "call_function" or nd.target not in (aten.mm.default, aten.addmm.default):
            continue
        v = nd.meta.get("val")
        a = nd.args[-2].meta.get("val") if isinstance(nd.args[-2], Node) else None
        if isinstance(v, torch.Tensor) and v.dtype == torch.bfloat16 and v.dim() == 2 and \
                isinstance(a, torch.Tensor) and a.dim() == 2:
            carriers.append((nd, 2.0 * v.shape[0] * v.shape[1] * a.shape[1]))
    gbps = float(os.environ.get("EDB_PF_GBPS", "300"))
    BLK = 16384
    need = sorted(uses, key=lambda ph: first_use[ph])
    start_of_carriers = order[carriers[0][0]] if carriers else float("inf")
    initial = [ph for ph in need if first_use[ph] < start_of_carriers]
    queue = deque([ph, 0] for ph in need if ph not in initial)
    late = {}
    deps = {ph: [] for ph in uses}

    def item(ph, done, take):
        shard, full, nbytes = bufs[ph]
        if my_index is None:
            return (shard.offset + done, full.offset + done, take, nbytes, 0)
        return (full.offset + done, full.offset + done, take, nbytes, nbytes)

    for nd, flops in carriers:
        budget = flops / 9e14 * gbps * 1e9 / max(1, n - 1) * 1.0
        items = []
        while queue and len(items) < 4:
            ph, done = queue[0]
            if order[nd] >= first_use[ph]:
                late.setdefault(ph, []).append(item(ph, done, bufs[ph][2] - done))
                queue.popleft()
                continue
            left = bufs[ph][2] - done
            take = left if left <= budget else max(BLK, int(budget) // BLK * BLK)
            take = min(take, left)
            items.append(item(ph, done, take))
            deps[ph].append(nd)
            budget -= take
            if take == left:
                queue.popleft()
            else:
                queue[0][1] = done + take
            if budget < BLK:
                break
        if items:
            nd.meta["edb_pf"] = {"group": list(ranks), "items": items}
    for ph, done in queue:
        late.setdefault(ph, []).append(item(ph, done, bufs[ph][2] - done))
    if initial:
        first_node = next(nd for nd in graph.nodes if nd.op != "placeholder")
        with graph.inserting_before(first_node):
            graph.call_function(ops.ag_prefetch, args=(initial[0], list(ranks)),
                                kwargs={"_items": [item(ph, 0, bufs[ph][2]) for ph in initial]})
    for ph, items in late.items():
        g0 = min(gathered_nodes[ph], key=lambda g: order[g])
        with graph.inserting_before(g0):
            graph.call_function(ops.ag_prefetch, args=(ph, list(ranks)), kwargs={"_items": items})
    for ph, lst in gathered_nodes.items():
        for g in lst:
            g.args = (ph, list(ranks)) + tuple(dict.fromkeys(d for d in deps[ph] if order[d] < order[g]))
    graph.lint()
    gm.recompile()
    return rehomed, len(uses)


def insert_epoch_barriers(gm, ranks, ops=_default_ops):
    graph = gm.graph
    order = {nd: i for i, nd in enumerate(graph.nodes)}
    peer_touch = tuple(getattr(ops, k) for k in ("ag_mm", "mm_push", "ag_prefetch") if hasattr(ops, k))
    fused_nodes = [nd for nd in graph.nodes if nd.op == "call_function"
                   and (nd.target in peer_touch or "edb_pf" in nd.meta)]
    if not fused_nodes:
        return 0
    n_new = 0
    last_fused = max(fused_nodes, key=lambda nd: order[nd])
    barriers = [nd for nd in graph.nodes if nd.op == "call_function"
                and nd.target is ops.epoch_barrier]
    if not any(order[b_] > order[last_fused] for b_ in barriers):
        anchor = last_fused
        while anchor.next.op == "call_function" and anchor.next.target is operator.getitem \
                and anchor.next.args[0] is last_fused:
            anchor = anchor.next
        with graph.inserting_after(anchor):
            graph.call_function(ops.epoch_barrier, args=(anchor, list(ranks)))
        n_new += 1
    return n_new + ensure_end_barrier(gm, ranks, ops)


def ensure_end_barrier(gm, ranks, ops=_default_ops):
    graph = gm.graph
    out_node = next(nd for nd in graph.nodes if nd.op == "output")
    prev = out_node.prev
    if prev.op == "call_function" and prev.target is ops.epoch_barrier:
        return 0
    some = next((nd for nd in reversed(list(graph.nodes)) if nd.op == "call_function"
                 and isinstance(nd.meta.get("val"), torch.Tensor)), None)
    if some is None:
        some = next(nd for nd in graph.nodes if nd.op == "placeholder")
    with graph.inserting_before(out_node):
        graph.call_function(ops.epoch_barrier, args=(some, list(ranks)))
    gm.recompile()
    return 1


def fuse_collective_gemms(gm, io, rt, ranks, ops=_default_ops, my_index=None):
    import os
    graph = gm.graph
    n = len(ranks)
    if n <= 1:
        return {}, {"ag_mm": 0, "ag_pf": 0, "mm_rs": 0}
    order = {nd: i for i, nd in enumerate(graph.nodes)}
    rehomed = {}
    n_ag = n_rs = 0
    bf16 = torch.bfloat16
    epoch = os.environ.get("EDB_EPOCH", "1") == "1" and hasattr(ops, "epoch_barrier")
    n_pf = 0
    if epoch and os.environ.get("EDB_AG_PREFETCH", "1") == "1" and hasattr(ops, "gathered"):
        rehomed, n_pf = prefetch_param_gathers(gm, io, rt, ranks, ops, my_index=my_index)
        order = {nd: i for i, nd in enumerate(graph.nodes)}

    def val(nd):
        return nd.meta.get("val") if isinstance(nd, Node) else None

    for ag_s in [x for x in graph.nodes if x.op == "call_function" and x.target is ops.all_gather_start]:
        ph = ag_s.args[0]
        if not (isinstance(ph, Node) and ph.op == "placeholder" and ph in io.param_ph):
            continue
        if ag_s.args[1] != 0 or len(ag_s.users) != 1:
            continue
        ag_e = next(iter(ag_s.users))
        if ag_e.target is not ops.all_gather_end or len(ag_e.users) != 1:
            continue
        v = next(iter(ag_e.users))
        if v.target != aten.view.default or len(v.args[1]) != 2 or len(v.users) != 1:
            continue
        n_out, k_in = (int(d) for d in v.args[1])
        t = next(iter(v.users))
        if t.target != aten.t.default or not t.users:
            continue
        first = min(t.users, key=lambda u: order[u])
        if first.target == aten.addmm.default and first.args[2] is t and not first.kwargs:
            bias, x = first.args[0], first.args[1]
        elif first.target == aten.mm.default and first.args[1] is t:
            bias, x = None, first.args[0]
        else:
            continue
        xv, pv = val(x), val(ph)
        if xv is None or pv is None or xv.dtype != bf16 or pv.dtype != bf16 or xv.dim() != 2:
            continue
        if n_out % n or n_out % 128 or (n_out // n) % 8 or k_in % 8 or xv.shape[1] != k_in:
            continue
        if bias is not None and (val(bias) is None or val(bias).dim() != 1 or n_out % 8):
            continue
        shard = rehomed.get(ph.name) or rt.alloc(n_out // n * k_in * 2, align=1024)
        full = rt.alloc(n_out * k_in * 2, align=1024)
        rehomed[ph.name] = shard
        with graph.inserting_before(first):
            ag_kw = {"_buf": (shard.offset, full.offset)}
            if epoch:
                ag_kw["_epoch"] = 1
            fused = graph.call_function(ops.ag_mm, args=(x, ph, list(ranks), n_out, k_in, bias),
                                        kwargs=ag_kw)
            out = graph.call_function(operator.getitem, args=(fused, 0))
            wfull = graph.call_function(operator.getitem, args=(fused, 1))
            t_new = graph.call_function(aten.t.default, args=(wfull,))
        first.replace_all_uses_with(out)
        graph.erase_node(first)
        t.replace_all_uses_with(t_new)
        for dead in (t, v, ag_e, ag_s):
            graph.erase_node(dead)
        n_ag += 1

    defer = epoch or (os.environ.get("EDB_DEFER_RS", "0") == "1" and hasattr(ops, "mm_rs_push"))
    pushed = []
    for rs_s in [x for x in graph.nodes if x.op == "call_function" and x.target is ops.reduce_scatter_start]:
        f = rs_s.args[0]
        if rs_s.args[1] != "avg" or rs_s.args[2] != 0 or rs_s.kwargs:
            continue
        if not (isinstance(f, Node) and f.target == aten.flatten.using_ints and len(f.users) == 1):
            continue
        g = f.args[0]
        if not (isinstance(g, Node) and len(g.users) == 1):
            continue
        t_chain = []
        mm_node = g
        while mm_node.target == aten.t.default and isinstance(mm_node.args[0], Node) and \
                len(mm_node.args[0].users) == 1:
            t_chain.append(mm_node)
# ... 365 lines not shown
```

### include/edb.h

```cpp
#ifndef EDB_H_
#define EDB_H_

#include <stddef.h>
#include <stdint.h>

#ifdef __cplusplus
extern "C" {
#endif

#define EDB_VERSION 100
#define EDB_MAX_GROUP 8
#define EDB_MAX_GROUPS 16
#define EDB_IPC_HANDLE_BYTES 64

enum edb_dtype { EDB_F32 = 0, EDB_BF16 = 1, EDB_F16 = 2, EDB_F64 = 3, EDB_I32 = 4, EDB_I64 = 5 };
enum edb_redop { EDB_SUM = 0, EDB_MAX = 1, EDB_MIN = 2, EDB_AVG = 3 };


int edb_version(void);
const char* edb_last_error(void);

int edb_init(int rank, int world, int device, size_t heap_bytes);
int edb_finalize(void);
int edb_is_initialized(void);
int edb_health(void);
int edb_heap_info(void** base, size_t* bytes, size_t* user_offset);

int edb_ipc_export(void* handle_out);
int edb_ipc_attach(int peer_rank, const void* handle);
int edb_attach_local(int peer_rank, void* base);

int edb_group_create(const int* ranks, int n, int slot, int* gid_out);
int edb_group_info(int gid, int* n_out, int* my_index_out);

int edb_symm_alloc(size_t bytes, size_t align, uint64_t* offset_out);
int edb_symm_mark(uint64_t* mark_out);
int edb_symm_reset(uint64_t mark);


int edb_scatter(void* dst, const void* src, const int64_t* shape, int ndim, int dim,
                int num_chunks, int index, int elem_size, int64_t* dst_extent_out, void* stream);

int edb_copy(void* dst, const void* src, size_t bytes, void* stream);

int edb_box_copy_local(void* dst, const int64_t* dst_strides, const void* src,
                       const int64_t* src_strides, const int64_t* extents, int ndim, int elem_size,
                       void* stream);


int edb_all_gather(int gid, uint64_t dst_off, const void* src, const int64_t* local_shape, int ndim,
                   int dim, int elem_size, void* stream);

int edb_reduce_scatter(int gid, void* dst, uint64_t stage_off, const void* src,
                       const int64_t* shape, int ndim, int dim, int dtype, int redop,
                       float post_scale, int out_dtype, void* stream);

int edb_all_reduce(int gid, void* dst, uint64_t stage_off, uint64_t stage2_off, const void* src,
                   int64_t numel, int dtype, int redop, void* stream);

int edb_all_to_all(int gid, void* dst, uint64_t stage_off, const void* src,
                   const int64_t* local_shape, int ndim, int gather_dim, int scatter_dim,
                   int elem_size, void* stream);

int edb_box_exchange(int gid, void* dst, const int64_t* dst_shape, uint64_t stage_off,
                     const void* src, const int64_t* src_shape, int ndim, int elem_size, int nbox,
                     const int* peer, const int64_t* src_start, const int64_t* dst_start,
                     const int64_t* extents, const int64_t* peer_src_shapes, void* stream);

int edb_halo_exchange(int gid, void* dst, uint64_t stage_off, const void* src,
                      const int64_t* local_shape, int ndim, int dim, int halo, int elem_size,
                      void* stream);

int edb_symm_guard(int gid, void* stream);


int edb_gemm_bf16(void* C, const void* A, const void* B, const void* bias, int64_t M, int64_t N,
                  int64_t K, int64_t lda, int64_t ldb, int64_t ldc, int a_kmajor, int b_kmajor,
                  int accumulate_into_c, void* stream);

int edb_gemm_epi_bf16(void* C, const void* A, const void* B, const void* bias, const void* aux,
                      int64_t ld_aux, int epi_op, int64_t M, int64_t N, int64_t K, int64_t lda,
                      int64_t ldb, int64_t ldc, int a_kmajor, int b_kmajor, int gid, int n_items,
                      const uint64_t* src_offs, const uint64_t* dst_offs, const int64_t* bytes,
                      const int64_t* dst_strides, const int64_t* src_strides, void* stream);

int edb_ag_gemm_bf16(int gid, void* C, const void* A, const void* bias, uint64_t b_shard_off,
                     uint64_t b_full_off, int64_t M, int64_t N, int64_t K, int64_t lda, int64_t ldc,
                     void* stream);

int edb_gemm_rs_bf16(int gid, void* dst, uint64_t c_stage_off, const void* A, const void* B,
                     int64_t M, int64_t N, int64_t K, int64_t lda, int64_t ldb, int a_kmajor,
                     int b_kmajor, float post_scale, int out_dtype, void* stream);

int edb_gemm_rs_push_bf16(int gid, uint64_t recv_off, uint64_t state_off, const void* A,
                          const void* B, int64_t M, int64_t N, int64_t K, int64_t lda, int64_t ldb,
                          int a_kmajor, int b_kmajor, void* stream);
int edb_rs_finish(int gid, int n_items, void* const* dsts, const uint64_t* recv_offs,
                  const uint64_t* state_offs, const int64_t* chunk_bytes, float post_scale,
                  int out_dtype, void* stream);


int edb_epoch_barrier(int gid, void* stream);

int edb_ag_gemm_epoch_bf16(int gid, void* C, const void* A, const void* bias, uint64_t b_shard_off,
                           uint64_t b_full_off, int64_t M, int64_t N, int64_t K, int64_t lda,
                           int64_t ldc, void* stream);

int edb_all_gather_push(int gid, uint64_t dst_off, const void* src, const int64_t* local_shape,
                        int ndim, int dim, int elem_size, void* stream);
int edb_all_to_all_push(int gid, uint64_t dst_off, const void* src, const int64_t* local_shape,
                        int ndim, int gather_dim, int scatter_dim, int elem_size, void* stream);
int edb_reduce_scatter_push(int gid, void* dst, uint64_t recv_off, const void* src,
                            const int64_t* shape, int ndim, int dim, int dtype, int redop,
                            float post_scale, int out_dtype, void* stream);
int edb_all_reduce_push(int gid, uint64_t out_off, uint64_t recv_off, const void* src, int64_t numel,
                        int dtype, int redop, void* stream);

int edb_ag_prefetch(int gid, int n_items, const uint64_t* src_offs, const uint64_t* dst_offs,
                    const int64_t* bytes, const int64_t* dst_strides, const int64_t* src_strides,
                    void* stream);
int edb_gemm_pf_bf16(void* C, const void* A, const void* B, const void* bias, int64_t M, int64_t N,
                     int64_t K, int64_t lda, int64_t ldb, int64_t ldc, int a_kmajor, int b_kmajor,
                     int gid, int n_items, const uint64_t* src_offs, const uint64_t* dst_offs,
                     const int64_t* bytes, const int64_t* dst_strides, const int64_t* src_strides,
                     void* stream);

int edb_gemm_push_bf16(int gid, uint64_t recv_off, const void* A, const void* B, int64_t M,
                       int64_t N, int64_t K, int64_t lda, int64_t ldb, int a_kmajor, int b_kmajor,
                       void* stream);

int edb_rs_finish_local(int gid, int n_items, void* const* dsts, const uint64_t* recv_offs,
                        const int64_t* chunk_bytes, float post_scale, int out_dtype, void* stream);

int edb_layer_norm_fwd(void* y, void* mean, void* rstd, const void* x, const void* w, const void* b,
                       int64_t rows, int64_t H, float eps, int dtype, void* stream);
int edb_layer_norm_bwd(void* dx, void* dw, void* db, const void* dy, const void* x, const void* mean,
                       const void* rstd, const void* w, void* workspace, int64_t rows, int64_t H,
                       int dtype, void* stream);
int edb_layer_norm_bwd_add(void* dx, void* dw, void* db, const void* dy, const void* x,
                           const void* mean, const void* rstd, const void* w, const void* add_in,
                           void* workspace, int64_t rows, int64_t H, int dtype, void* stream);
int edb_layer_norm_bwd_workspace(int64_t H, size_t* bytes_out);

#define EDB_RMS_CAST_THEN_SCALE 0
#define EDB_RMS_FUSED 1
int edb_rms_norm_fwd(void* y, void* rstd, const void* x, const void* w, int64_t rows, int64_t H,
                     float eps, int mode, int dtype, void* stream);
int edb_rms_norm_bwd(void* dx, void* dw, const void* dy, const void* x, const void* rstd,
                     const void* w, const void* add_in, void* workspace, int64_t rows, int64_t H,
                     int mode, int dtype, void* stream);
int edb_rms_norm_bwd_workspace(int64_t H, size_t* bytes_out);

int edb_swiglu_fwd(void* out, const void* gate, const void* up, int64_t n, int dtype, void* stream);
int edb_swiglu_bwd(void* dgate, void* dup, const void* dy, const void* gate, const void* up,
                   int64_t n, int dtype, void* stream);

int edb_rope(void* y, const void* x, const void* cos, const void* sin, int64_t B, int64_t H,
             int64_t T, int64_t half, const int64_t* x_strides, const int64_t* y_strides,
             int64_t table_stride_t, int inverse, int dtype, void* stream);

int edb_embedding_fwd(void* y, const void* weight, const void* idx, const void* pos_weight,
                      const void* pos, int64_t rows, int64_t C, int64_t V, int64_t Vp, int64_t T,
                      int idx_dtype, int dtype, void* stream);
int edb_embedding_bwd(void* out, int64_t ld_out, const void* dy, int64_t ld_dy, const void* idx,
                      void* workspace, int64_t rows, int64_t C, int64_t V, int64_t padding_idx,
                      int accumulate, int idx_dtype, int dtype, void* stream);
int edb_embedding_bwd_workspace(int64_t rows, int64_t V, size_t* bytes_out);

int edb_colsum(void* out, const void* x, void* workspace, int64_t rows, int64_t cols, int64_t ld,
               int dtype, void* stream);
int edb_colsum_workspace(int64_t cols, size_t* bytes_out);

int edb_cross_entropy_fwd(float* loss, float* total_weight, float* lse, float* row_loss,
                          const void* logits, int64_t ld, const int64_t* target, int64_t rows,
                          int64_t vocab, int64_t ignore_index, int reduction, int dtype, void* stream);
int edb_cross_entropy_bwd(void* dlogits, int64_t ld_out, const void* logits, int64_t ld,
                          const int64_t* target, const float* lse, const float* grad_out,
                          const float* total_weight, int64_t rows, int64_t vocab,
                          int64_t ignore_index, int reduction, int dtype, void* stream);

int edb_sgd_momentum(int n, void* const* params, const void* const* grads, void* const* bufs,
                     const int64_t* numels, float mu, float grad_alpha, float neg_lr, int dtype,
                     void* stream);
int edb_sgd_momentum_scaled(int n, void* const* params, const void* const* grads, void* const* bufs,
                            const int64_t* numels, float mu, float grad_alpha, float neg_lr,
                            const void* grad_scale, int dtype, void* stream);

#define EDB_SUMSQ_RAW 0
#define EDB_SUMSQ_NORM 1
int edb_grad_sumsq(int n, const void* const* grads, const int64_t* numels, void* out,
                   void* workspace, int mode, int dtype, void* stream);
int edb_grad_sumsq_workspace(int n, const int64_t* numels, int dtype, size_t* bytes_out);
int edb_multi_scale_(int n, void* const* grads, const int64_t* numels, const void* coef, int dtype,
                     void* stream);


int edb_set_option(const char* name, int64_t value);
int edb_get_option(const char* name, int64_t* value_out);
uint64_t edb_launch_count(void);

#define EDB_OK 0
#define EDB_E_INVALID 1
#define EDB_E_UNSUPPORTED 2
#define EDB_E_CUDA 3
#define EDB_E_STATE 4

#ifdef __cplusplus
}
#endif
#endif
```

Before: 341.5.

## Add native wgmma/TMA causal flash attention kernels and fold QKV grad concat

Adds a custom Hopper causal flash-attention forward and backward (TMA loads, multi-stage mbarrier pipeline, wgmma) and rewires SDPA flash/cudnn nodes in the traced graph to call it when head dim is 64 and shapes fit. The backward can write dq/dk/dv directly into a fused [B,T,3C] buffer, removing the transpose/view/cat chain and its extra copy. The aim is to replace the aten SDPA kernels with a specialised kernel and save memory traffic. Unsupported shapes fall back to aten; the risk is that the hand-written kernel is slower than FlashAttention/cuDNN.

```diff
diff --git a/easydist_b200/_lib.py b/easydist_b200/_lib.py
--- a/easydist_b200/_lib.py
+++ b/easydist_b200/_lib.py
@@ -112,6 +112,11 @@
     "edb_embedding_bwd": (c_int, [c_void_p, c_int64, c_void_p, c_int64, c_void_p, c_void_p, c_int64,
                                   c_int64, c_int64, c_int64, c_int, c_int, c_int, c_void_p]),
     "edb_embedding_bwd_workspace": (c_int, [c_int64, c_int64, POINTER(c_size_t)]),
+    "edb_attn_fwd": (c_int, [c_void_p, _I64P, c_void_p, c_void_p, _I64P, c_void_p, _I64P, c_void_p,
+                             _I64P, c_int, c_int, c_int, c_void_p]),
+    "edb_attn_bwd": (c_int, [c_void_p, _I64P, c_void_p, _I64P, c_void_p, _I64P, c_void_p, c_void_p,
+                             _I64P, c_void_p, _I64P, c_void_p, _I64P, c_void_p, _I64P, c_void_p,
+                             _I64P, c_void_p, c_int, c_int, c_int, c_void_p]),
     "edb_colsum": (c_int,[c_void_p, c_void_p, c_void_p, c_int64, c_int64, c_int64, c_int, c_void_p]),
     "edb_colsum_workspace": (c_int, [c_int64, POINTER(c_size_t)]),
     "edb_cross_entropy_fwd": (c_int, [c_void_p, c_void_p, c_void_p, c_void_p, c_void_p, c_int64,
diff --git a/easydist_b200/api.py b/easydist_b200/api.py
--- a/easydist_b200/api.py
+++ b/easydist_b200/api.py
@@ -140,6 +140,7 @@
         info["rope_nodes"] = counts["rope"]
         info["clip_nodes"] = counts["clip"]
         info["embed_nodes"] = counts["embed"]
+        info["attn_nodes"] = counts["attn"]
         if ranks is not None and len(ranks) > 1 and (push or info.get("fused")):
             try:
                 rep = lowering.verify_epoch_protocol(gm, ops, len(ranks))
diff --git a/easydist_b200/attn.py b/easydist_b200/attn.py
--- /dev/null
+++ b/easydist_b200/attn.py
@@ -0,0 +1,105 @@
+import torch
+from torch._subclasses.fake_tensor import FakeTensor
+
+from . import _lib
+from ._lib import check
+from .norm import _stream
+
+aten = torch.ops.aten
+_stats = {"edb_attn_fwd": 0, "edb_attn_bwd": 0, "aten_attn": 0}
+
+
+def stats():
+    return dict(_stats)
+
+
+def reset_stats():
+    for k in _stats:
+        _stats[k] = 0
+
+
+def _strides(t):
+    return (_lib.c_int64 * 3)(*t.stride()[:3])
+
+
+def _view_ok(t):
+    return t.stride(3) == 1 and all(s % 8 == 0 and s > 0 for s in t.stride()[:3]) \
+        and t.data_ptr() % 16 == 0
+
+
+def native_ok(q, k, v):
+    if isinstance(q, FakeTensor) or not q.is_cuda or q.dim() != 4:
+        return False
+    B, H, T, D = q.shape
+    return (D == 64 and T % 64 == 0 and T > 0 and B * H <= 65535
+            and all(x.dtype == torch.bfloat16 and x.device == q.device and x.shape == q.shape
+                    and _view_ok(x) for x in (q, k, v)))
+
+
+def _count_aten(t):
+    if not isinstance(t, FakeTensor):
+        _stats["aten_attn"] += 1
+
+
+def attention_fwd(q, k, v):
+    B, H, T, D = q.shape
+    out = q.new_empty((B, T, H, D)).transpose(1, 2)
+    lse = torch.empty((B, H, T), dtype=torch.float32, device=q.device)
+    check(_lib.load().edb_attn_fwd(out.data_ptr(), _strides(out), lse.data_ptr(), q.data_ptr(),
+                                   _strides(q), k.data_ptr(), _strides(k), v.data_ptr(),
+                                   _strides(v), B, H, T, _stream(q)))
+    _stats["edb_attn_fwd"] += 1
+    return out, lse
+
+
+def qkv_grad_views(dqkv, H):
+    B, T, C3 = dqkv.shape
+    C = C3 // 3
+    return tuple(dqkv[:, :, i * C:(i + 1) * C].view(B, T, H, C // H).transpose(1, 2)
+                 for i in range(3))
+
+
+def attention_bwd(dout, q, k, v, out, lse, dqkv=None):
+    B, H, T, D = q.shape
+    if dqkv is None:
+        grads = tuple(q.new_empty((B, T, H, D)).transpose(1, 2) for _ in range(3))
+    else:
+        grads = qkv_grad_views(dqkv, H)
+    if dout.stride(3) != 1 or dout.data_ptr() % 16 or any(s % 8 for s in dout.stride()[:3]):
+        dout = dout.contiguous()
+    if not _view_ok(out):
+        out = out.contiguous()
+    dsum = torch.empty((B, H, T), dtype=torch.float32, device=q.device)
+    dq, dk, dv = grads
+    check(_lib.load().edb_attn_bwd(dq.data_ptr(), _strides(dq), dk.data_ptr(), _strides(dk),
+                                   dv.data_ptr(), _strides(dv), dsum.data_ptr(), dout.data_ptr(),
+                                   _strides(dout), q.data_ptr(), _strides(q), k.data_ptr(),
+                                   _strides(k), v.data_ptr(), _strides(v), out.data_ptr(),
+                                   _strides(out), lse.data_ptr(), B, H, T, _stream(q)))
+    _stats["edb_attn_bwd"] += 1
+    return grads
+
+
+def sdpa_fwd(op, *args, **kwargs):
+    q, k, v = args[:3]
+    if not native_ok(q, k, v):
+        _count_aten(q)
+        return op(*args, **kwargs)
+    out, lse = attention_fwd(q, k, v)
+    return (out, lse) + (None,) * (len(op._schema.returns) - 2)
+
+
+def sdpa_bwd(op, *args, fold_qkv=False, **kwargs):
+    dout, q, k, v, out, lse = args[:6]
+    if not native_ok(q, k, v):
+        _count_aten(q)
+        grads = tuple(op(*args, **kwargs)[:3])
+        if not fold_qkv:
+            return grads
+        B, H, T, D = q.shape
+        return grads + (torch.cat([g.transpose(1, 2).reshape(B, T, H * D) for g in grads], 2),)
+    if not fold_qkv:
+        return attention_bwd(dout, q, k, v, out, lse)
+    B, H, T, D = q.shape
+    dqkv = q.new_empty((B, T, 3 * H * D))
+    return attention_bwd(dout, q, k, v, out, lse, dqkv) + (dqkv,)
diff --git a/easydist_b200/build.py b/easydist_b200/build.py
--- a/easydist_b200/build.py
+++ b/easydist_b200/build.py
@@ -12,8 +12,8 @@
 LIB_PATH = os.path.join(HERE, "libedb.so")
 BUILD_DIR = os.path.join(HERE, "csrc", "_build")
 
-HEADERS = ["edb_internal.cuh", "edb_vec.cuh"]
-SOURCES = ["edb_runtime.cu", "edb_reshard.cu", "edb_ll.cu", "edb_norm.cu", "edb_rms.cu", "edb_rope.cu", "edb_embed.cu", "edb_loss.cu", "edb_optim.cu", "edb_clip.cu", "edb_gemm.cu"]
+HEADERS = ["edb_internal.cuh", "edb_vec.cuh", "edb_wgmma.cuh"]
+SOURCES = ["edb_runtime.cu", "edb_reshard.cu", "edb_ll.cu", "edb_norm.cu", "edb_rms.cu", "edb_rope.cu", "edb_embed.cu", "edb_loss.cu", "edb_optim.cu", "edb_clip.cu", "edb_gemm.cu", "edb_attn.cu"]
 
 ARCH = "arch=compute_90a,code=sm_90a"
 
diff --git a/easydist_b200/csrc/edb_attn.cu b/easydist_b200/csrc/edb_attn.cu
--- /dev/null
+++ b/easydist_b200/csrc/edb_attn.cu
@@ -0,0 +1,513 @@
+#include <cuda.h>
+#include <cuda_bf16.h>
+
+#include "edb_internal.cuh"
+#include "edb_wgmma.cuh"
+
+namespace edb {
+
+namespace {
+
+constexpr int kAttnTile = 64;
+constexpr int kAttnThreads = 160;
+constexpr int kAttnTileBytes = kAttnTile * kAttnTile * 2;
+constexpr int kAttnStages = 3;
+constexpr int kAttnSmem = (2 + 2 * kAttnStages) * kAttnTileBytes + 1024 + 128;
+constexpr float kLog2e = 1.4426950408889634f;
+
+struct AttnMaps {
+  CUtensorMap a, b;
+  CUtensorMap c, d;
+};
+
+struct AttnOut {
+  __nv_bfloat16* p0;
+  __nv_bfloat16* p1;
+  int64_t s0[3], s1[3];
+};
+
+struct AttnArgs {
+  float* lse;
+  const float* dsum;
+  int H, T, n_tiles;
+  float scale_log2;
+  float scale;
+};
+
+__device__ __forceinline__ void tma_load_4d(const CUtensorMap* map, uint64_t* bar, void* smem, int t,
+                                            int h, int b) {
+  asm volatile(
+      "cp.async.bulk.tensor.4d.shared::cluster.global.mbarrier::complete_tx::bytes [%0], [%1, {%3, "
+      "%4, %5, %6}], [%2];" ::"r"(smem_u32(smem)),
+      "l"(map), "r"(smem_u32(bar)), "r"(0), "r"(t), "r"(h), "r"(b)
+      : "memory");
+}
+
+template <int TA, int TB>
+__device__ __forceinline__ void wgmma_ss64(float* d, uint64_t da, uint64_t db, uint32_t scale_d) {
+  asm volatile(
+      "{\n"
+      ".reg .pred p;\n"
+      "setp.ne.b32 p, %34, 0;\n"
+      "wgmma.mma_async.sync.aligned.m64n64k16.f32.bf16.bf16 "
+      "{%0, %1, %2, %3, %4, %5, %6, %7, %8, %9, %10, %11, %12, %13, %14, %15, "
+      "%16, %17, %18, %19, %20, %21, %22, %23, %24, %25, %26, %27, %28, %29, %30, %31}, "
+      "%32, %33, p, 1, 1, %35, %36;\n"
+      "}\n"
+      : "+f"(d[0]), "+f"(d[1]), "+f"(d[2]), "+f"(d[3]), "+f"(d[4]), "+f"(d[5]), "+f"(d[6]), "+f"(d[7]),
+        "+f"(d[8]), "+f"(d[9]), "+f"(d[10]), "+f"(d[11]), "+f"(d[12]), "+f"(d[13]), "+f"(d[14]), "+f"(d[15]),
+        "+f"(d[16]), "+f"(d[17]), "+f"(d[18]), "+f"(d[19]), "+f"(d[20]), "+f"(d[21]), "+f"(d[22]), "+f"(d[23]),
+        "+f"(d[24]), "+f"(d[25]), "+f"(d[26]), "+f"(d[27]), "+f"(d[28]), "+f"(d[29]), "+f"(d[30]), "+f"(d[31])
+      : "l"(da), "l"(db), "r"(scale_d), "n"(TA), "n"(TB));
+}
+
+__device__ __forceinline__ void wgmma_rs64(float* d, const uint32_t* a, uint64_t db, uint32_t scale_d) {
+  asm volatile(
+      "{\n"
+      ".reg .pred p;\n"
+      "setp.ne.b32 p, %37, 0;\n"
+      "wgmma.mma_async.sync.aligned.m64n64k16.f32.bf16.bf16 "
+      "{%0, %1, %2, %3, %4, %5, %6, %7, %8, %9, %10, %11, %12, %13, %14, %15, "
+      "%16, %17, %18, %19, %20, %21, %22, %23, %24, %25, %26, %27, %28, %29, %30, %31}, "
+      "{%32, %33, %34, %35}, %36, p, 1, 1, 1;\n"
+      "}\n"
+      : "+f"(d[0]), "+f"(d[1]), "+f"(d[2]), "+f"(d[3]), "+f"(d[4]), "+f"(d[5]), "+f"(d[6]), "+f"(d[7]),
+        "+f"(d[8]), "+f"(d[9]), "+f"(d[10]), "+f"(d[11]), "+f"(d[12]), "+f"(d[13]), "+f"(d[14]), "+f"(d[15]),
+        "+f"(d[16]), "+f"(d[17]), "+f"(d[18]), "+f"(d[19]), "+f"(d[20]), "+f"(d[21]), "+f"(d[22]), "+f"(d[23]),
+        "+f"(d[24]), "+f"(d[25]), "+f"(d[26]), "+f"(d[27]), "+f"(d[28]), "+f"(d[29]), "+f"(d[30]), "+f"(d[31])
+      : "r"(a[0]), "r"(a[1]), "r"(a[2]), "r"(a[3]), "l"(db), "r"(scale_d));
+}
+
+__device__ __forceinline__ void mma_abt(float* c, uint32_t a, uint32_t b) {
+#pragma unroll
+  for (int k = 0; k < 4; ++k)
+    wgmma_ss64<0, 0>(c, make_smem_desc(a + k * 32, 16, 1024), make_smem_desc(b + k * 32, 16, 1024),
+                     k > 0);
+}
+
+__device__ __forceinline__ void mma_rb(float* c, const uint32_t* a, uint32_t b, bool fresh) {
+#pragma unroll
+  for (int k = 0; k < 4; ++k)
+    wgmma_rs64(c, a + 4 * k, make_smem_desc(b + k * 16 * 128, 8192, 1024), !(fresh && k == 0));
+}
+
+__device__ __forceinline__ uint32_t pack_bf16(float lo, float hi) {
+  __nv_bfloat162 v = __floats2bfloat162_rn(lo, hi);
+  return *reinterpret_cast<uint32_t*>(&v);
+}
+
+__device__ __forceinline__ void to_frag(uint32_t* a, const float* c) {
+#pragma unroll
+  for (int i = 0; i < 16; ++i) a[i] = pack_bf16(c[2 * i], c[2 * i + 1]);
+}
+
+__device__ __forceinline__ int frag_row(int tid, int i) { return 16 * (tid / 32) + (tid % 32) / 4 + 8 * ((i / 2) % 2); }
+__device__ __forceinline__ int frag_col(int tid, int i) { return 8 * (i / 4) + 2 * (tid % 4) + i % 2; }
+
+__device__ __forceinline__ void store_tile(__nv_bfloat16* base, const int64_t* s, int b, int h, int t0,
+                                           int tid, const float* c, float mul) {
+  __nv_bfloat16* p = base + (int64_t)b * s[0] + (int64_t)h * s[1];
+#pragma unroll
+  for (int i = 0; i < 32; i += 2) {
+    const int64_t r = t0 + frag_row(tid, i);
+    *reinterpret_cast<__nv_bfloat162*>(p + r * s[2] + frag_col(tid, i)) =
+        __floats2bfloat162_rn(c[i] * mul, c[i + 1] * mul);
+  }
+}
+
+__device__ __forceinline__ uint8_t* stage_tile(uint8_t* stages, int s, int i) {
+  return stages + (2 * s + i) * kAttnTileBytes;
+}
+
+struct SmemLayout {
+  uint8_t* fixed0;
+  uint8_t* fixed1;
+  uint8_t* stages;
+  uint64_t* fixed_bar;
+  uint64_t* full;
+  uint64_t* empty;
+};
+
+__device__ __forceinline__ SmemLayout carve(uint8_t* raw) {
+  uint8_t* base = (uint8_t*)(((uintptr_t)raw + 1023) & ~(uintptr_t)1023);
+  SmemLayout L;
+  L.fixed0 = base;
+  L.fixed1 = base + kAttnTileBytes;
+  L.stages = base + 2 * kAttnTileBytes;
+  uint64_t* bars = (uint64_t*)(base + (2 + 2 * kAttnStages) * kAttnTileBytes);
+  L.fixed_bar = bars;
+  L.full = bars + 1;
+  L.empty = bars + 1 + kAttnStages;
+  return L;
+}
+
+__device__ __forceinline__ void produce(const AttnMaps& m, const SmemLayout& L, int nfixed, int t_fixed,
+                                        int t_first, int count, int h, int b) {
+  mbar_expect_tx(L.fixed_bar, nfixed * kAttnTileBytes);
+  tma_load_4d(&m.a, L.fixed_bar, L.fixed0, t_fixed, h, b);
+  if (nfixed == 2) tma_load_4d(&m.b, L.fixed_bar, L.fixed1, t_fixed, h, b);
+  for (int n = 0; n < count; ++n) {
+    const int s = n % kAttnStages;
+    if (n >= kAttnStages) mbar_wait(&L.empty[s], ((n / kAttnStages) - 1) & 1);
+    mbar_expect_tx(&L.full[s], 2 * kAttnTileBytes);
+    tma_load_4d(&m.c, &L.full[s], stage_tile(L.stages, s, 0), t_first + kAttnTile * n, h, b);
+    tma_load_4d(&m.d, &L.full[s], stage_tile(L.stages, s, 1), t_first + kAttnTile * n, h, b);
+  }
+}
+
+__device__ __forceinline__ void init_bars(const SmemLayout& L) {
+  if (threadIdx.x == 0) {
+    mbar_init(L.fixed_bar, 1);
+    for (int s = 0; s < kAttnStages; ++s) {
+      mbar_init(&L.full[s], 1);
+      mbar_init(&L.empty[s], 4);
+    }
+    fence_barrier_init();
+  }
+  __syncthreads();
+}
+
+__device__ __forceinline__ void release(const SmemLayout& L, int s, int tid) {
+  if ((tid & 31) == 0) mbar_arrive(&L.empty[s]);
+}
+
+__device__ __forceinline__ void tile_of(const AttnArgs& a, int& b, int& h, int& tile) {
+  b = blockIdx.x / a.H;
+  h = blockIdx.x % a.H;
+  tile = a.n_tiles - 1 - blockIdx.y;
+}
+
+__global__ void __launch_bounds__(kAttnThreads, 3) k_attn_fwd(const __grid_constant__ AttnMaps m,
+                                                           const AttnOut o, const AttnArgs a) {
+  extern __shared__ uint8_t smem_raw[];
+  const SmemLayout L = carve(smem_raw);
+  int b, h, qt;
+  tile_of(a, b, h, qt);
+  const int nkv = qt + 1;
+  init_bars(L);
+  const int tid = threadIdx.x;
+  if (tid >= 128) {
+    if (tid == 128) produce(m, L, 1, qt * kAttnTile, 0, nkv, h, b);
+    return;
+  }
+  float acc[32], s[32];
+  uint32_t pf[16];
+  float mrow[2] = {-INFINITY, -INFINITY}, lrow[2] = {0.f, 0.f};
+  mbar_wait(L.fixed_bar, 0);
+  const uint32_t q = smem_u32(L.fixed0);
+  mbar_wait(&L.full[0], 0);
+  wgmma_fence();
+  mma_abt(s, q, smem_u32(stage_tile(L.stages, 0, 0)));
+  wgmma_commit();
+  wgmma_wait<0>();
+  for (int j = 0; j < nkv; ++j) {
+    const int st = j % kAttnStages;
+    wgmma_wait<1>();
+    const bool diag = j == qt;
+    float corr[2], pr[32];
+#pragma unroll
+    for (int r = 0; r < 2; ++r) {
+      float mx = mrow[r];
+#pragma unroll
+      for (int i = 0; i < 32; ++i) {
+        if ((i / 2) % 2 != r) continue;
+        float v = s[i] * a.scale_log2;
+        if (diag && frag_col(tid, i) > frag_row(tid, i)) v = -INFINITY;
+        pr[i] = v;
+        mx = fmaxf(mx, v);
+      }
+      mx = fmaxf(mx, __shfl_xor_sync(0xffffffffu, mx, 1));
+      mx = fmaxf(mx, __shfl_xor_sync(0xffffffffu, mx, 2));
+      corr[r] = exp2f(mrow[r] - mx);
+      mrow[r] = mx;
+      float sum = 0.f;
+#pragma unroll
+      for (int i = 0; i < 32; ++i) {
+        if ((i / 2) % 2 != r) continue;
+        pr[i] = exp2f(pr[i] - mx);
+        sum += pr[i];
+      }
+      lrow[r] = lrow[r] * corr[r] + sum;
+    }
+    wgmma_wait<0>();
+    if (j > 0) release(L, (j - 1) % kAttnStages, tid);
+#pragma unroll
+    for (int i = 0; i < 32; ++i) acc[i] *= corr[(i / 2) % 2];
+    to_frag(pf, pr);
+    if (j + 1 < nkv) {
+      const int sn = (j + 1) % kAttnStages;
+      mbar_wait(&L.full[sn], ((j + 1) / kAttnStages) & 1);
+      wgmma_fence();
+      mma_abt(s, q, smem_u32(stage_tile(L.stages, sn, 0)));
+      wgmma_commit();
+    }
+    wgmma_fence();
+    mma_rb(acc, pf, smem_u32(stage_tile(L.stages, st, 1)), j == 0);
+    wgmma_commit();
+  }
+  wgmma_wait<0>();
+  float inv[2];
+#pragma unroll
+  for (int r = 0; r < 2; ++r) {
+    float l = lrow[r];
+    l += __shfl_xor_sync(0xffffffffu, l, 1);
+    l += __shfl_xor_sync(0xffffffffu, l, 2);
+    inv[r] = 1.f / l;
+    if (tid % 4 == 0) {
+      const int row = qt * kAttnTile + frag_row(tid, 2 * r);
+      a.lse[((int64_t)b * a.H + h) * a.T + row] = mrow[r] * 0.6931471805599453f + logf(l);
+    }
+  }
+#pragma unroll
+  for (int i = 0; i < 32; ++i) acc[i] *= inv[(i / 2) % 2];
+  store_tile(o.p0, o.s0, b, h, qt * kAttnTile, tid, acc, 1.f);
+}
+
+__global__ void __launch_bounds__(256) k_attn_bwd_dot(float* dsum, const __nv_bfloat16* dout,
+                                                      const __nv_bfloat16* out, AttnOut st, int H,
+                                                      int T, int64_t rows) {
+  const int64_t row = ((int64_t)blockIdx.x * 256 + threadIdx.x) / 8;
+  const int part = threadIdx.x % 8;
+  float acc = 0.f;
+  if (row < rows) {
+    const int64_t t = row % T, bh = row / T, h = bh % H, b = bh / H;
+    const uint4 x = *reinterpret_cast<const uint4*>(dout + b * st.s0[0] + h * st.s0[1] + t * st.s0[2] + 8 * part);
+    const uint4 y = *reinterpret_cast<const uint4*>(out + b * st.s1[0] + h * st.s1[1] + t * st.s1[2] + 8 * part);
+    const __nv_bfloat162* xv = reinterpret_cast<const __nv_bfloat162*>(&x);
+    const __nv_bfloat162* yv = reinterpret_cast<const __nv_bfloat162*>(&y);
+#pragma unroll
+    for (int i = 0; i < 4; ++i) {
+      const float2 xf = __bfloat1622float2(xv[i]), yf = __bfloat1622float2(yv[i]);
+      acc += xf.x * yf.x + xf.y * yf.y;
+    }
+  }
+  acc += __shfl_xor_sync(0xffffffffu, acc, 1);
+  acc += __shfl_xor_sync(0xffffffffu, acc, 2);
+  acc += __shfl_xor_sync(0xffffffffu, acc, 4);
+  if (row < rows && part == 0) dsum[row] = acc;
+}
+
+__global__ void __launch_bounds__(kAttnThreads) k_attn_bwd_dkdv(const __grid_constant__ AttnMaps m,
+                                                                const AttnOut o, const AttnArgs a) {
+  extern __shared__ uint8_t smem_raw[];
+  const SmemLayout L = carve(smem_raw);
+  const int b = blockIdx.x / a.H, h = blockIdx.x % a.H;
+  const int kt = blockIdx.y;
+  const int nq = a.n_tiles - kt;
+  init_bars(L);
+  const int tid = threadIdx.x;
+  if (tid >= 128) {
+    if (tid == 128) produce(m, L, 2, kt * kAttnTile, kt * kAttnTile, nq, h, b);
+    return;
+  }
+  float dk[32], dv[32], s[32], dp[32];
+  uint32_t pf[16], df[16];
+#pragma unroll
+  for (int i = 0; i < 32; ++i) dk[i] = dv[i] = 0.f;
+  const int64_t bh = (int64_t)b * a.H + h;
+  const float* lse = a.lse + bh * a.T;
+  const float* dsum = a.dsum + bh * a.T;
+  mbar_wait(L.fixed_bar, 0);
+  const uint32_t kk = smem_u32(L.fixed0), vv = smem_u32(L.fixed1);
+  for (int n = 0; n < nq; ++n) {
+    const int st = n % kAttnStages;
+    const int q0 = (kt + n) * kAttnTile;
+    mbar_wait(&L.full[st], (n / kAttnStages) & 1);
+    const uint32_t qs = smem_u32(stage_tile(L.stages, st, 0)), dos = smem_u32(stage_tile(L.stages, st, 1));
+    wgmma_fence();
+    mma_abt(s, kk, qs);
+    mma_abt(dp, vv, dos);
+    wgmma_commit();
+    float l2[16], dd[16];
+#pragma unroll
+    for (int c = 0; c < 16; ++c) {
+      const int col = q0 + 8 * (c / 2) + 2 * (tid % 4) + (c % 2);
+      l2[c] = lse[col] * kLog2e;
+      dd[c] = dsum[col];
+    }
+    wgmma_wait<0>();
+    const bool diag = n == 0;
+#pragma unroll
+    for (int i = 0; i < 32; ++i) {
+      const int c = 2 * (i / 4) + (i % 2);
+      float p = exp2f(s[i] * a.scale_log2 - l2[c]);
+      if (diag && frag_col(tid, i) < frag_row(tid, i)) p = 0.f;
+      s[i] = p;
+      dp[i] = p * (dp[i] - dd[c]);
+    }
+    to_frag(pf, s);
+    to_frag(df, dp);
+    wgmma_fence();
+    mma_rb(dv, pf, dos, false);
+    mma_rb(dk, df, qs, false);
+    wgmma_commit();
+    wgmma_wait<0>();
+    release(L, st, tid);
+  }
+  const int t0 = kt * kAttnTile;
+  store_tile(o.p0, o.s0, b, h, t0, tid, dk, a.scale);
+  store_tile(o.p1, o.s1, b, h, t0, tid, dv, 1.f);
+}
+
+__global__ void __launch_bounds__(kAttnThreads) k_attn_bwd_dq(const __grid_constant__ AttnMaps m,
+                                                              const AttnOut o, const AttnArgs a) {
+  extern __shared__ uint8_t smem_raw[];
+  const SmemLayout L = carve(smem_raw);
+  int b, h, qt;
+  tile_of(a, b, h, qt);
+  const int nkv = qt + 1;
+  init_bars(L);
+  const int tid = threadIdx.x;
+  if (tid >= 128) {
+    if (tid == 128) produce(m, L, 2, qt * kAttnTile, 0, nkv, h, b);
+    return;
+  }
+  float dq[32], s[32], dp[32];
+  uint32_t df[16];
+#pragma unroll
+  for (int i = 0; i < 32; ++i) dq[i] = 0.f;
+  const int64_t bh = (int64_t)b * a.H + h;
+  float l2[2], dd[2];
+#pragma unroll
+  for (int r = 0; r < 2; ++r) {
+    const int row = qt * kAttnTile + frag_row(tid, 2 * r);
+    l2[r] = a.lse[bh * a.T + row] * kLog2e;
+    dd[r] = a.dsum[bh * a.T + row];
+  }
+  mbar_wait(L.fixed_bar, 0);
+  const uint32_t qs = smem_u32(L.fixed0), dos = smem_u32(L.fixed1);
+  for (int j = 0; j < nkv; ++j) {
+    const int st = j % kAttnStages;
+    mbar_wait(&L.full[st], (j / kAttnStages) & 1);
+    const uint32_t ks = smem_u32(stage_tile(L.stages, st, 0)), vs = smem_u32(stage_tile(L.stages, st, 1));
+    wgmma_fence();
+    mma_abt(s, qs, ks);
+    mma_abt(dp, dos, vs);
+    wgmma_commit();
+    wgmma_wait<0>();
+    const bool diag = j == qt;
+#pragma unroll
+    for (int i = 0; i < 32; ++i) {
+      const int r = (i / 2) % 2;
+      float p = exp2f(s[i] * a.scale_log2 - l2[r]);
+      if (diag && frag_col(tid, i) > frag_row(tid, i)) p = 0.f;
+      dp[i] = p * (dp[i] - dd[r]);
+    }
+    to_frag(df, dp);
+    wgmma_fence();
+    mma_rb(dq, df, ks, false);
+    wgmma_commit();
+    wgmma_wait<0>();
+    release(L, st, tid);
+  }
+  store_tile(o.p0, o.s0, b, h, qt * kAttnTile, tid, dq, a.scale);
+}
+
+typedef CUresult (*EncodeTiledFn)(CUtensorMap*, CUtensorMapDataType, cuuint32_t, void*,
+                                  const cuuint64_t*, const cuuint64_t*, const cuuint32_t*,
+                                  const cuuint32_t*, CUtensorMapInterleave, CUtensorMapSwizzle,
+                                  CUtensorMapL2promotion, CUtensorMapFloatOOBfill);
+
+int attn_tmap(CUtensorMap* map, const void* base, const int64_t* s, int B, int H, int T) {
+  static EncodeTiledFn fn = nullptr;
+  if (!fn) {
+    void* p = nullptr;
+    cudaDriverEntryPointQueryResult q;
+    if (cudaGetDriverEntryPoint("cuTensorMapEncodeTiled", &p, cudaEnableDefault, &q) != cudaSuccess ||
+        q != cudaDriverEntryPointSuccess)
+      return set_error(EDB_E_CUDA, "cuTensorMapEncodeTiled entry point not available");
+    fn = reinterpret_cast<EncodeTiledFn>(p);
+  }
+  if ((uintptr_t)base & 15) return set_error(EDB_E_UNSUPPORTED, "attention: operand not 16-byte aligned");
+  for (int i = 0; i < 3; ++i)
+    if (s[i] % 8 || s[i] <= 0) return set_error(EDB_E_UNSUPPORTED, "attention: stride %lld", (long long)s[i]);
+  cuuint64_t dims[4] = {64, (cuuint64_t)T, (cuuint64_t)H, (cuuint64_t)B};
+  cuuint64_t strides[3] = {(cuuint64_t)s[2] * 2, (cuuint64_t)s[1] * 2, (cuuint64_t)s[0] * 2};
+  cuuint32_t box[4] = {64, 64, 1, 1};
+  cuuint32_t estr[4] = {1, 1, 1, 1};
+  CUresult rc = fn(map, CU_TENSOR_MAP_DATA_TYPE_BFLOAT16, 4, const_cast<void*>(base), dims, strides, box,
+                   estr, CU_TENSOR_MAP_INTERLEAVE_NONE, CU_TENSOR_MAP_SWIZZLE_128B,
+                   CU_TENSOR_MAP_L2_PROMOTION_L2_256B, CU_TENSOR_MAP_FLOAT_OOB_FILL_NONE);
+  if (rc != CUDA_SUCCESS) return set_error(EDB_E_CUDA, "attention: cuTensorMapEncodeTiled failed (%d)", (int)rc);
+  return EDB_OK;
+}
+
+int attn_check(int B, int H, int T, const char* who) {
+  if (B < 1 || H < 1 || T < kAttnTile || T % kAttnTile || (int64_t)B * H > 65535)
+    return set_error(EDB_E_UNSUPPORTED, "%s: B=%d H=%d T=%d (T a multiple of 64)", who, B, H, T);
+  return EDB_OK;
+}
+
+typedef void (*AttnKernel)(const AttnMaps, const AttnOut, const AttnArgs);
+
+int attn_launch(AttnKernel kern, bool& configured, const char* name, const AttnMaps& m, const AttnOut& o,
+                const AttnArgs& a, int BH, cudaStream_t st) {
+  if (!configured) {
+    EDB_CUDA(cudaFuncSetAttribute(kern, cudaFuncAttributeMaxDynamicSharedMemorySize, kAttnSmem));
+    configured = true;
+  }
+  kern<<<dim3(BH, a.n_tiles), kAttnThreads, kAttnSmem, st>>>(m, o, a);
+  count_launch();
+  return cuda_check(cudaGetLastError(), name);
+}
+
+bool cfg_fwd = false, cfg_dkdv = false, cfg_dq = false;
+
+}
+
+}
+
+using namespace edb;
+
+extern "C" int edb_attn_fwd(void* out, const int64_t* out_strides, float* lse, const void* q,
+                            const int64_t* q_strides, const void* k, const int64_t* k_strides,
+                            const void* v, const int64_t* v_strides, int B, int H, int T, void* stream) {
+  int rc = attn_check(B, H, T, "attn_fwd");
+  if (rc) return rc;
+  AttnMaps m;
+  if ((rc = attn_tmap(&m.a, q, q_strides, B, H, T)) || (rc = attn_tmap(&m.c, k, k_strides, B, H, T)) ||
+      (rc = attn_tmap(&m.d, v, v_strides, B, H, T)))
+    return rc;
+  m.b = m.a;
+  AttnOut o = {};
+  o.p0 = (__nv_bfloat16*)out;
+  for (int i = 0; i < 3; ++i) o.s0[i] = out_strides[i];
+  AttnArgs a = {lse, nullptr, H, T, T / kAttnTile, 0.125f * kLog2e, 0.125f};
+  return attn_launch(k_attn_fwd, cfg_fwd, "k_attn_fwd launch", m, o, a, B * H, (cudaStream_t)stream);
+}
+
+extern "C" int edb_attn_bwd(void* dq, const int64_t* dq_strides, void* dk, const int64_t* dk_strides,
+                            void* dv, const int64_t* dv_strides, float* dsum, const void* dout,
+                            const int64_t* dout_strides, const void* q, const int64_t* q_strides,
+                            const void* k, const int64_t* k_strides, const void* v,
+                            const int64_t* v_strides, const void* out, const int64_t* out_strides,
+                            const float* lse, int B, int H, int T, void* stream) {
+  int rc = attn_check(B, H, T, "attn_bwd");
+  if (rc) return rc;
+  if (((uintptr_t)out & 15) || out_strides[0] % 8 || out_strides[1] % 8 || out_strides[2] % 8)
+    return set_error(EDB_E_UNSUPPORTED, "attn_bwd: out not 16-byte aligned");
+  CUtensorMap tq, tk, tv, tdo;
+  if ((rc = attn_tmap(&tq, q, q_strides, B, H, T)) || (rc = attn_tmap(&tk, k, k_strides, B, H, T)) ||
+      (rc = attn_tmap(&tv, v, v_strides, B, H, T)) || (rc = attn_tmap(&tdo, dout, dout_strides, B, H, T)))
+    return rc;
+  cudaStream_t st = (cudaStream_t)stream;
+  AttnOut od = {};
+  for (int i = 0; i < 3; ++i) od.s0[i] = dout_strides[i], od.s1[i] = out_strides[i];
+  const int64_t rows = (int64_t)B * H * T;
+  k_attn_bwd_dot<<<(unsigned)((rows * 8 + 255) / 256), 256, 0, st>>>(
+      dsum, (const __nv_bfloat16*)dout, (const __nv_bfloat16*)out, od, H, T, rows);
+  count_launch();
+  if ((rc = cuda_check(cudaGetLastError(), "k_attn_bwd_dot launch"))) return rc;
+  AttnArgs a = {const_cast<float*>(lse), dsum, H, T, T / kAttnTile, 0.125f * kLog2e, 0.125f};
+  AttnMaps m1 = {tk, tv, tq, tdo};
+  AttnOut o1 = {};
+  o1.p0 = (__nv_bfloat16*)dk;
+  o1.p1 = (__nv_bfloat16*)dv;
+  for (int i = 0; i < 3; ++i) o1.s0[i] = dk_strides[i], o1.s1[i] = dv_strides[i];
+  if ((rc = attn_launch(k_attn_bwd_dkdv, cfg_dkdv, "k_attn_bwd_dkdv launch", m1, o1, a, B * H, st))) return rc;
+  AttnMaps m2 = {tq, tdo, tk, tv};
+  AttnOut o2 = {};
+  o2.p0 = (__nv_bfloat16*)dq;
+  for (int i = 0; i < 3; ++i) o2.s0[i] = dq_strides[i];
+  return attn_launch(k_attn_bwd_dq, cfg_dq, "k_attn_bwd_dq launch", m2, o2, a, B * H, st);
+}
diff --git a/easydist_b200/csrc/edb_gemm.cu b/easydist_b200/csrc/edb_gemm.cu
--- a/easydist_b200/csrc/edb_gemm.cu
+++ b/easydist_b200/csrc/edb_gemm.cu
@@ -2,6 +2,7 @@
 #include <cuda_bf16.h>
 
 #include "edb_internal.cuh"
+#include "edb_wgmma.cuh"
 
 namespace edb {
 
@@ -22,164 +23,8 @@
       kStages * kStageBytes + kEpiBufs * kEpiBufBytes + 1024  + 256 ;
 };
 
-
-__device__ __forceinline__ uint32_t smem_u32(const void* p) {
-  return static_cast<uint32_t>(__cvta_generic_to_shared(p));
-}
-__device__ __forceinline__ void mbar_init(uint64_t* bar, uint32_t count) {
-  asm volatile("mbarrier.init.shared::cta.b64 [%0], %1;" ::"r"(smem_u32(bar)), "r"(count));
-}
-__device__ __forceinline__ void mbar_expect_tx(uint64_t* bar, uint32_t bytes) {
-  asm volatile("mbarrier.arrive.expect_tx.shared::cta.b64 _, [%0], %1;" ::"r"(smem_u32(bar)),
-               "r"(bytes)
-               : "memory");
-}
-__device__ __forceinline__ void mbar_arrive(uint64_t* bar) {
-  asm volatile("mbarrier.arrive.shared::cta.b64 _, [%0];" ::"r"(smem_u32(bar)) : "memory");
-}
-__device__ __forceinline__ bool mbar_try_wait(uint32_t addr, uint32_t parity) {
-  uint32_t ok;
-  asm volatile(
-      "{\n"
-      ".reg .pred p;\n"
-      "mbarrier.try_wait.parity.shared::cta.b64 p, [%1], %2;\n"
-      "selp.u32 %0, 1, 0, p;\n"
-      "}\n"
-      : "=r"(ok)
-      : "r"(addr), "r"(parity)
-      : "memory");
-  return ok != 0;
-}
-__device__ __forceinline__ void mbar_wait(uint64_t* bar, uint32_t parity) {
-  const uint32_t addr = smem_u32(bar);
-  if (mbar_try_wait(addr, parity)) return;
-  const uint64_t t0 = globaltimer_ns();
-  uint32_t spins = 0;
-  while (!mbar_try_wait(addr, parity)) {
-    if ((++spins & 0xfff) == 0 && globaltimer_ns() - t0 > 4000000000ull) {
-      asm volatile("trap;");
-    }
-  }
-}
-__device__ __forceinline__ void fence_barrier_init() {
-  asm volatile("fence.mbarrier_init.release.cluster;" ::: "memory");
-}
-__device__ __forceinline__ void fence_proxy_async() {
-  asm volatile("fence.proxy.async.shared::cta;" ::: "memory");
-}
-__device__ __forceinline__ void tma_load_2d(const CUtensorMap* map, uint64_t* bar, void* smem,
-                                            int c0, int c1) {
-  asm volatile(
-      "cp.async.bulk.tensor.2d.shared::cluster.global.mbarrier::complete_tx::bytes [%0], [%1, {%3, "
-      "%4}], [%2];" ::"r"(smem_u32(smem)),
-      "l"(map), "r"(smem_u32(bar)), "r"(c0), "r"(c1)
-      : "memory");
-}
-__device__ __forceinline__ void tma_store_2d(const CUtensorMap* map, const void* smem, int c0,
-                                             int c1) {
-  asm volatile(
-      "cp.async.bulk.tensor.2d.global.shared::cta.bulk_group [%0, {%2, %3}], [%1];" ::"l"(map),
-      "r"(smem_u32(smem)), "r"(c0), "r"(c1)
-      : "memory");
-}
-__device__ __forceinline__ void tma_store_commit() {
-  asm volatile("cp.async.bulk.commit_group;" ::: "memory");
-}
-template <int N> __device__ __forceinline__ void tma_store_wait_read() {
-  asm volatile("cp.async.bulk.wait_group.read %0;" ::"n"(N) : "memory");
-}
-__device__ __forceinline__ void tma_store_wait_all() {
-  asm volatile("cp.async.bulk.wait_group 0;" ::: "memory");
-}
 __device__ __forceinline__ void epi_bar_sync() {
   asm volatile("bar.sync 1, %0;" ::"n"(kConsumerThreads) : "memory");
-}
-__device__ __forceinline__ void prefetch_tmap(const CUtensorMap* map) {
-  asm volatile("prefetch.tensormap [%0];" ::"l"(map) : "memory");
-}
-__device__ __forceinline__ void wgmma_fence() {
-  asm volatile("wgmma.fence.sync.aligned;" ::: "memory");
-}
-__device__ __forceinline__ void wgmma_commit() {
-  asm volatile("wgmma.commit_group.sync.aligned;" ::: "memory");
-}
-template <int N> __device__ __forceinline__ void wgmma_wait() {
-  asm volatile("wgmma.wait_group.sync.aligned %0;" ::"n"(N) : "memory");
-}
-
-template <int TA, int TB>
-__device__ __forceinline__ void wgmma_m64n128k16(float* d, uint64_t desc_a, uint64_t desc_b,
-                                                  uint32_t scale_d) {
-  asm volatile(
-      "{\n"
-      ".reg .pred p;\n"
-      "setp.ne.b32 p, %66, 0;\n"
-      "wgmma.mma_async.sync.aligned.m64n128k16.f32.bf16.bf16 "
-      "{"
-      "%0, %1, %2, %3, %4, %5, %6, %7, %8, %9, %10, %11, %12, %13, %14, %15, "
-      "%16, %17, %18, %19, %20, %21, %22, %23, %24, %25, %26, %27, %28, %29, %30, %31, "
-      "%32, %33, %34, %35, %36, %37, %38, %39, %40, %41, %42, %43, %44, %45, %46, %47, "
-      "%48, %49, %50, %51, %52, %53, %54, %55, %56, %57, %58, %59, %60, %61, %62, %63"
-      "}, %64, %65, p, 1, 1, %67, %68;\n"
-      "}\n"
-      : "+f"(d[0]), "+f"(d[1]), "+f"(d[2]), "+f"(d[3]), "+f"(d[4]), "+f"(d[5]), "+f"(d[6]), "+f"(d[7]),
-        "+f"(d[8]), "+f"(d[9]), "+f"(d[10]), "+f"(d[11]), "+f"(d[12]), "+f"(d[13]), "+f"(d[14]), "+f"(d[15]),
-        "+f"(d[16]), "+f"(d[17]), "+f"(d[18]), "+f"(d[19]), "+f"(d[20]), "+f"(d[21]), "+f"(d[22]), "+f"(d[23]),
-        "+f"(d[24]), "+f"(d[25]), "+f"(d[26]), "+f"(d[27]), "+f"(d[28]), "+f"(d[29]), "+f"(d[30]), "+f"(d[31]),
-        "+f"(d[32]), "+f"(d[33]), "+f"(d[34]), "+f"(d[35]), "+f"(d[36]), "+f"(d[37]), "+f"(d[38]), "+f"(d[39]),
-        "+f"(d[40]), "+f"(d[41]), "+f"(d[42]), "+f"(d[43]), "+f"(d[44]), "+f"(d[45]), "+f"(d[46]), "+f"(d[47]),
-        "+f"(d[48]), "+f"(d[49]), "+f"(d[50]), "+f"(d[51]), "+f"(d[52]), "+f"(d[53]), "+f"(d[54]), "+f"(d[55]),
-        "+f"(d[56]), "+f"(d[57]), "+f"(d[58]), "+f"(d[59]), "+f"(d[60]), "+f"(d[61]), "+f"(d[62]), "+f"(d[63])
-      : "l"(desc_a), "l"(desc_b), "r"(scale_d), "n"(TA), "n"(TB));
-}
-
-template <int TA, int TB>
-__device__ __forceinline__ void wgmma_m64n256k16(float* d, uint64_t desc_a, uint64_t desc_b,
-                                                  uint32_t scale_d) {
-  asm volatile(
-      "{\n"
-      ".reg .pred p;\n"
-      "setp.ne.b32 p, %130, 0;\n"
-      "wgmma.mma_async.sync.aligned.m64n256k16.f32.bf16.bf16 "
-      "{"
-      "%0, %1, %2, %3, %4, %5, %6, %7, %8, %9, %10, %11, %12, %13, %14, %15, "
-      "%16, %17, %18, %19, %20, %21, %22, %23, %24, %25, %26, %27, %28, %29, %30, %31, "
-      "%32, %33, %34, %35, %36, %37, %38, %39, %40, %41, %42, %43, %44, %45, %46, %47, "
-      "%48, %49, %50, %51, %52, %53, %54, %55, %56, %57, %58, %59, %60, %61, %62, %63, "
-      "%64, %65, %66, %67, %68, %69, %70, %71, %72, %73, %74, %75, %76, %77, %78, %79, "
-      "%80, %81, %82, %83, %84, %85, %86, %87, %88, %89, %90, %91, %92, %93, %94, %95, "
-      "%96, %97, %98, %99, %100, %101, %102, %103, %104, %105, %106, %107, %108, %109, %110, %111, "
-      "%112, %113, %114, %115, %116, %117, %118, %119, %120, %121, %122, %123, %124, %125, %126, %127"
-      "}, %128, %129, p, 1, 1, %131, %132;\n"
-      "}\n"
-      : "+f"(d[0]), "+f"(d[1]), "+f"(d[2]), "+f"(d[3]), "+f"(d[4]), "+f"(d[5]), "+f"(d[6]), "+f"(d[7]),
-        "+f"(d[8]), "+f"(d[9]), "+f"(d[10]), "+f"(d[11]), "+f"(d[12]), "+f"(d[13]), "+f"(d[14]), "+f"(d[15]),
-        "+f"(d[16]), "+f"(d[17]), "+f"(d[18]), "+f"(d[19]), "+f"(d[20]), "+f"(d[21]), "+f"(d[22]), "+f"(d[23]),
-        "+f"(d[24]), "+f"(d[25]), "+f"(d[26]), "+f"(d[27]), "+f"(d[28]), "+f"(d[29]), "+f"(d[30]), "+f"(d[31]),
-        "+f"(d[32]), "+f"(d[33]), "+f"(d[34]), "+f"(d[35]), "+f"(d[36]), "+f"(d[37]), "+f"(d[38]), "+f"(d[39]),
-        "+f"(d[40]), "+f"(d[41]), "+f"(d[42]), "+f"(d[43]), "+f"(d[44]), "+f"(d[45]), "+f"(d[46]), "+f"(d[47]),
-        "+f"(d[48]), "+f"(d[49]), "+f"(d[50]), "+f"(d[51]), "+f"(d[52]), "+f"(d[53]), "+f"(d[54]), "+f"(d[55]),
-        "+f"(d[56]), "+f"(d[57]), "+f"(d[58]), "+f"(d[59]), "+f"(d[60]), "+f"(d[61]), "+f"(d[62]), "+f"(d[63]),
-        "+f"(d[64]), "+f"(d[65]), "+f"(d[66]), "+f"(d[67]), "+f"(d[68]), "+f"(d[69]), "+f"(d[70]), "+f"(d[71]),
-        "+f"(d[72]), "+f"(d[73]), "+f"(d[74]), "+f"(d[75]), "+f"(d[76]), "+f"(d[77]), "+f"(d[78]), "+f"(d[79]),
-        "+f"(d[80]), "+f"(d[81]), "+f"(d[82]), "+f"(d[83]), "+f"(d[84]), "+f"(d[85]), "+f"(d[86]), "+f"(d[87]),
-        "+f"(d[88]), "+f"(d[89]), "+f"(d[90]), "+f"(d[91]), "+f"(d[92]), "+f"(d[93]), "+f"(d[94]), "+f"(d[95]),
-        "+f"(d[96]), "+f"(d[97]), "+f"(d[98]), "+f"(d[99]), "+f"(d[100]), "+f"(d[101]), "+f"(d[102]), "+f"(d[103]),
-        "+f"(d[104]), "+f"(d[105]), "+f"(d[106]), "+f"(d[107]), "+f"(d[108]), "+f"(d[109]), "+f"(d[110]), "+f"(d[111]),
-        "+f"(d[112]), "+f"(d[113]), "+f"(d[114]), "+f"(d[115]), "+f"(d[116]), "+f"(d[117]), "+f"(d[118]), "+f"(d[119]),
-        "+f"(d[120]), "+f"(d[121]), "+f"(d[122]), "+f"(d[123]), "+f"(d[124]), "+f"(d[125]), "+f"(d[126]), "+f"(d[127])
-      : "l"(desc_a), "l"(desc_b), "r"(scale_d), "n"(TA), "n"(TB));
-}
-
-
-__device__ __forceinline__ uint64_t make_smem_desc(uint32_t smem_addr, uint32_t lbo_bytes,
-                                                   uint32_t sbo_bytes) {
-  uint64_t d = 0;
-  d |= (uint64_t)((smem_addr >> 4) & 0x3fff);
-  d |= (uint64_t)((lbo_bytes >> 4) & 0x3fff) << 16;
-  d |= (uint64_t)((sbo_bytes >> 4) & 0x3fff) << 32;
-  d |= (uint64_t)1 << 62;
-  return d;
 }
 
 struct GemmParams {
@@ -904,12 +749,6 @@
 constexpr int kGemm2Threads = 384;
 constexpr int kGemm2EpiBufBytes = 64 * 64 * 2;
 
-template <int R> __device__ __forceinline__ void setmaxnreg_dec() {
-  asm volatile("setmaxnreg.dec.sync.aligned.u32 %0;" ::"n"(R));
-}
-template <int R> __device__ __forceinline__ void setmaxnreg_inc() {
-  asm volatile("setmaxnreg.inc.sync.aligned.u32 %0;" ::"n"(R));
-}
 __device__ __forceinline__ void wg_bar_sync(int wg) {
   if (wg == 0) asm volatile("bar.sync 1, 128;" ::: "memory");
   else asm volatile("bar.sync 2, 128;" ::: "memory");
diff --git a/easydist_b200/csrc/edb_wgmma.cuh b/easydist_b200/csrc/edb_wgmma.cuh
--- /dev/null
+++ b/easydist_b200/csrc/edb_wgmma.cuh
@@ -0,0 +1,172 @@
+#pragma once
+#include <cuda.h>
+#include <cstdint>
+
+#include "edb_internal.cuh"
+
+namespace edb {
+
+__device__ __forceinline__ uint32_t smem_u32(const void* p) {
+  return static_cast<uint32_t>(__cvta_generic_to_shared(p));
+}
+__device__ __forceinline__ void mbar_init(uint64_t* bar, uint32_t count) {
+  asm volatile("mbarrier.init.shared::cta.b64 [%0], %1;" ::"r"(smem_u32(bar)), "r"(count));
+}
+__device__ __forceinline__ void mbar_expect_tx(uint64_t* bar, uint32_t bytes) {
+  asm volatile("mbarrier.arrive.expect_tx.shared::cta.b64 _, [%0], %1;" ::"r"(smem_u32(bar)),
+               "r"(bytes)
+               : "memory");
+}
+__device__ __forceinline__ void mbar_arrive(uint64_t* bar) {
+  asm volatile("mbarrier.arrive.shared::cta.b64 _, [%0];" ::"r"(smem_u32(bar)) : "memory");
+}
+__device__ __forceinline__ bool mbar_try_wait(uint32_t addr, uint32_t parity) {
+  uint32_t ok;
+  asm volatile(
+      "{\n"
+      ".reg .pred p;\n"
+      "mbarrier.try_wait.parity.shared::cta.b64 p, [%1], %2;\n"
+      "selp.u32 %0, 1, 0, p;\n"
+      "}\n"
+      : "=r"(ok)
+      : "r"(addr), "r"(parity)
+      : "memory");
+  return ok != 0;
+}
+__device__ __forceinline__ void mbar_wait(uint64_t* bar, uint32_t parity) {
+  const uint32_t addr = smem_u32(bar);
+  if (mbar_try_wait(addr, parity)) return;
+  const uint64_t t0 = globaltimer_ns();
+  uint32_t spins = 0;
+  while (!mbar_try_wait(addr, parity)) {
+    if ((++spins & 0xfff) == 0 && globaltimer_ns() - t0 > 4000000000ull) {
+      asm volatile("trap;");
+    }
+  }
+}
+__device__ __forceinline__ void fence_barrier_init() {
+  asm volatile("fence.mbarrier_init.release.cluster;" ::: "memory");
+}
+__device__ __forceinline__ void fence_proxy_async() {
+  asm volatile("fence.proxy.async.shared::cta;" ::: "memory");
+}
+__device__ __forceinline__ void tma_load_2d(const CUtensorMap* map, uint64_t* bar, void* smem,
+                                            int c0, int c1) {
+  asm volatile(
+      "cp.async.bulk.tensor.2d.shared::cluster.global.mbarrier::complete_tx::bytes [%0], [%1, {%3, "
+      "%4}], [%2];" ::"r"(smem_u32(smem)),
+      "l"(map), "r"(smem_u32(bar)), "r"(c0), "r"(c1)
+      : "memory");
+}
+__device__ __forceinline__ void tma_store_2d(const CUtensorMap* map, const void* smem, int c0,
+                                             int c1) {
+  asm volatile(
+      "cp.async.bulk.tensor.2d.global.shared::cta.bulk_group [%0, {%2, %3}], [%1];" ::"l"(map),
+      "r"(smem_u32(smem)), "r"(c0), "r"(c1)
+      : "memory");
+}
+__device__ __forceinline__ void tma_store_commit() {
+  asm volatile("cp.async.bulk.commit_group;" ::: "memory");
+}
+template <int N> __device__ __forceinline__ void tma_store_wait_read() {
+  asm volatile("cp.async.bulk.wait_group.read %0;" ::"n"(N) : "memory");
+}
+__device__ __forceinline__ void tma_store_wait_all() {
+  asm volatile("cp.async.bulk.wait_group 0;" ::: "memory");
+}
+__device__ __forceinline__ void prefetch_tmap(const CUtensorMap* map) {
+  asm volatile("prefetch.tensormap [%0];" ::"l"(map) : "memory");
+}
+__device__ __forceinline__ void wgmma_fence() {
+  asm volatile("wgmma.fence.sync.aligned;" ::: "memory");
+}
+__device__ __forceinline__ void wgmma_commit() {
+  asm volatile("wgmma.commit_group.sync.aligned;" ::: "memory");
+}
+template <int N> __device__ __forceinline__ void wgmma_wait() {
+  asm volatile("wgmma.wait_group.sync.aligned %0;" ::"n"(N) : "memory");
+}
+
+template <int TA, int TB>
+__device__ __forceinline__ void wgmma_m64n128k16(float* d, uint64_t desc_a, uint64_t desc_b,
+                                                  uint32_t scale_d) {
+  asm volatile(
+      "{\n"
+      ".reg .pred p;\n"
+      "setp.ne.b32 p, %66, 0;\n"
+      "wgmma.mma_async.sync.aligned.m64n128k16.f32.bf16.bf16 "
+      "{"
+      "%0, %1, %2, %3, %4, %5, %6, %7, %8, %9, %10, %11, %12, %13, %14, %15, "
+      "%16, %17, %18, %19, %20, %21, %22, %23, %24, %25, %26, %27, %28, %29, %30, %31, "
+      "%32, %33, %34, %35, %36, %37, %38, %39, %40, %41, %42, %43, %44, %45, %46, %47, "
+      "%48, %49, %50, %51, %52, %53, %54, %55, %56, %57, %58, %59, %60, %61, %62, %63"
+      "}, %64, %65, p, 1, 1, %67, %68;\n"
+      "}\n"
+      : "+f"(d[0]), "+f"(d[1]), "+f"(d[2]), "+f"(d[3]), "+f"(d[4]), "+f"(d[5]), "+f"(d[6]), "+f"(d[7]),
+        "+f"(d[8]), "+f"(d[9]), "+f"(d[10]), "+f"(d[11]), "+f"(d[12]), "+f"(d[13]), "+f"(d[14]), "+f"(d[15]),
+        "+f"(d[16]), "+f"(d[17]), "+f"(d[18]), "+f"(d[19]), "+f"(d[20]), "+f"(d[21]), "+f"(d[22]), "+f"(d[23]),
+        "+f"(d[24]), "+f"(d[25]), "+f"(d[26]), "+f"(d[27]), "+f"(d[28]), "+f"(d[29]), "+f"(d[30]), "+f"(d[31]),
+        "+f"(d[32]), "+f"(d[33]), "+f"(d[34]), "+f"(d[35]), "+f"(d[36]), "+f"(d[37]), "+f"(d[38]), "+f"(d[39]),
+        "+f"(d[40]), "+f"(d[41]), "+f"(d[42]), "+f"(d[43]), "+f"(d[44]), "+f"(d[45]), "+f"(d[46]), "+f"(d[47]),
+        "+f"(d[48]), "+f"(d[49]), "+f"(d[50]), "+f"(d[51]), "+f"(d[52]), "+f"(d[53]), "+f"(d[54]), "+f"(d[55]),
+        "+f"(d[56]), "+f"(d[57]), "+f"(d[58]), "+f"(d[59]), "+f"(d[60]), "+f"(d[61]), "+f"(d[62]), "+f"(d[63])
+      : "l"(desc_a), "l"(desc_b), "r"(scale_d), "n"(TA), "n"(TB));
+}
+
+template <int TA, int TB>
+__device__ __forceinline__ void wgmma_m64n256k16(float* d, uint64_t desc_a, uint64_t desc_b,
+                                                  uint32_t scale_d) {
+  asm volatile(
+      "{\n"
+      ".reg .pred p;\n"
+      "setp.ne.b32 p, %130, 0;\n"
+      "wgmma.mma_async.sync.aligned.m64n256k16.f32.bf16.bf16 "
+      "{"
+      "%0, %1, %2, %3, %4, %5, %6, %7, %8, %9, %10, %11, %12, %13, %14, %15, "
+      "%16, %17, %18, %19, %20, %21, %22, %23, %24, %25, %26, %27, %28, %29, %30, %31, "
+      "%32, %33, %34, %35, %36, %37, %38, %39, %40, %41, %42, %43, %44, %45, %46, %47, "
+      "%48, %49, %50, %51, %52, %53, %54, %55, %56, %57, %58, %59, %60, %61, %62, %63, "
+      "%64, %65, %66, %67, %68, %69, %70, %71, %72, %73, %74, %75, %76, %77, %78, %79, "
+      "%80, %81, %82, %83, %84, %85, %86, %87, %88, %89, %90, %91, %92, %93, %94, %95, "
+      "%96, %97, %98, %99, %100, %101, %102, %103, %104, %105, %106, %107, %108, %109, %110, %111, "
+      "%112, %113, %114, %115, %116, %117, %118, %119, %120, %121, %122, %123, %124, %125, %126, %127"
+      "}, %128, %129, p, 1, 1, %131, %132;\n"
+      "}\n"
+      : "+f"(d[0]), "+f"(d[1]), "+f"(d[2]), "+f"(d[3]), "+f"(d[4]), "+f"(d[5]), "+f"(d[6]), "+f"(d[7]),
+        "+f"(d[8]), "+f"(d[9]), "+f"(d[10]), "+f"(d[11]), "+f"(d[12]), "+f"(d[13]), "+f"(d[14]), "+f"(d[15]),
+        "+f"(d[16]), "+f"(d[17]), "+f"(d[18]), "+f"(d[19]), "+f"(d[20]), "+f"(d[21]), "+f"(d[22]), "+f"(d[23]),
+        "+f"(d[24]), "+f"(d[25]), "+f"(d[26]), "+f"(d[27]), "+f"(d[28]), "+f"(d[29]), "+f"(d[30]), "+f"(d[31]),
+        "+f"(d[32]), "+f"(d[33]), "+f"(d[34]), "+f"(d[35]), "+f"(d[36]), "+f"(d[37]), "+f"(d[38]), "+f"(d[39]),
+        "+f"(d[40]), "+f"(d[41]), "+f"(d[42]), "+f"(d[43]), "+f"(d[44]), "+f"(d[45]), "+f"(d[46]), "+f"(d[47]),
+        "+f"(d[48]), "+f"(d[49]), "+f"(d[50]), "+f"(d[51]), "+f"(d[52]), "+f"(d[53]), "+f"(d[54]), "+f"(d[55]),
+        "+f"(d[56]), "+f"(d[57]), "+f"(d[58]), "+f"(d[59]), "+f"(d[60]), "+f"(d[61]), "+f"(d[62]), "+f"(d[63]),
+        "+f"(d[64]), "+f"(d[65]), "+f"(d[66]), "+f"(d[67]), "+f"(d[68]), "+f"(d[69]), "+f"(d[70]), "+f"(d[71]),
+        "+f"(d[72]), "+f"(d[73]), "+f"(d[74]), "+f"(d[75]), "+f"(d[76]), "+f"(d[77]), "+f"(d[78]), "+f"(d[79]),
+        "+f"(d[80]), "+f"(d[81]), "+f"(d[82]), "+f"(d[83]), "+f"(d[84]), "+f"(d[85]), "+f"(d[86]), "+f"(d[87]),
+        "+f"(d[88]), "+f"(d[89]), "+f"(d[90]), "+f"(d[91]), "+f"(d[92]), "+f"(d[93]), "+f"(d[94]), "+f"(d[95]),
+        "+f"(d[96]), "+f"(d[97]), "+f"(d[98]), "+f"(d[99]), "+f"(d[100]), "+f"(d[101]), "+f"(d[102]), "+f"(d[103]),
+        "+f"(d[104]), "+f"(d[105]), "+f"(d[106]), "+f"(d[107]), "+f"(d[108]), "+f"(d[109]), "+f"(d[110]), "+f"(d[111]),
+        "+f"(d[112]), "+f"(d[113]), "+f"(d[114]), "+f"(d[115]), "+f"(d[116]), "+f"(d[117]), "+f"(d[118]), "+f"(d[119]),
+        "+f"(d[120]), "+f"(d[121]), "+f"(d[122]), "+f"(d[123]), "+f"(d[124]), "+f"(d[125]), "+f"(d[126]), "+f"(d[127])
+      : "l"(desc_a), "l"(desc_b), "r"(scale_d), "n"(TA), "n"(TB));
+}
+
+
+__device__ __forceinline__ uint64_t make_smem_desc(uint32_t smem_addr, uint32_t lbo_bytes,
+                                                   uint32_t sbo_bytes) {
+  uint64_t d = 0;
+  d |= (uint64_t)((smem_addr >> 4) & 0x3fff);
+  d |= (uint64_t)((lbo_bytes >> 4) & 0x3fff) << 16;
+  d |= (uint64_t)((sbo_bytes >> 4) & 0x3fff) << 32;
+  d |= (uint64_t)1 << 62;
+  return d;
+}
+
+template <int R> __device__ __forceinline__ void setmaxnreg_dec() {
+  asm volatile("setmaxnreg.dec.sync.aligned.u32 %0;" ::"n"(R));
+}
+template <int R> __device__ __forceinline__ void setmaxnreg_inc() {
+  asm volatile("setmaxnreg.inc.sync.aligned.u32 %0;" ::"n"(R));
+}
+
+}
diff --git a/easydist_b200/lowering.py b/easydist_b200/lowering.py
--- a/easydist_b200/lowering.py
+++ b/easydist_b200/lowering.py
@@ -1784,6 +1784,85 @@
                 frontier.append(u)
 
 
+_SDPA_PAIRS = {
+    aten._scaled_dot_product_flash_attention.default:
+        aten._scaled_dot_product_flash_attention_backward.default,
+    aten._scaled_dot_product_flash_attention_for_cpu.default:
+        aten._scaled_dot_product_flash_attention_for_cpu_backward.default,
+    aten._scaled_dot_product_cudnn_attention.default:
+        aten._scaled_dot_product_cudnn_attention_backward.default,
+}
+
+
+def _sdpa_plain(nd):
+    sch = nd.target._schema
+    a = {x.name: x.default_value if x.has_default_value() else None for x in sch.arguments}
+    a.update({x.name: v for x, v in zip(sch.arguments, nd.args)})
+    a.update(nd.kwargs)
+    return a.get("is_causal") is True and a.get("dropout_p") in (0, 0.0) and a.get("scale") is None \
+        and a.get("attn_mask") is None and a.get("attn_bias") is None \
+        and not a.get("return_debug_mask", False)
+
+
+def _getitem(nd, i):
+    return next((u for u in nd.users if u.target is operator.getitem and u.args[1] == i), None)
+
+
+def _fold_qkv_cat(bwd):
+    chain, srcs = [], []
+    for i in range(3):
+        g = _getitem(bwd, i)
+        t = _only_user(g) if g is not None and len(g.users) == 1 else None
+        if not (_call(t, aten.transpose.int) and tuple(t.args[1:]) in ((1, 2), (2, 1))):
+            return None
+        vw = _only_user(t)
+        if not (_call(vw, aten.view.default) and len(vw.args[1]) == 3):
+            return None
+        chain += [vw, t, g]
+        srcs.append(vw)
+    cat = _only_user(srcs[0])
+    if not (_call(cat, aten.cat.default) and list(cat.args[0]) == srcs
+            and (cat.args[1] if len(cat.args) > 1 else 0) in (2, -1)
+            and all(_only_user(x) is cat for x in srcs)):
+        return None
+    return cat, chain
+
+
+def fuse_attention(gm):
+    from . import attn
+    graph = gm.graph
+    nf = nb = ncat = 0
+    for fwd in list(graph.nodes):
+        if not _call(fwd, *_SDPA_PAIRS) or not _sdpa_plain(fwd):
+            continue
+        out, lse = _getitem(fwd, 0), _getitem(fwd, 1)
+        bwd_t = _SDPA_PAIRS[fwd.target]
+        bwds = [u for u in (out.users if out is not None else ())
+                if _call(u, bwd_t) and len(u.args) >= 6 and u.args[4] is out and u.args[5] is lse
+                and tuple(u.args[1:4]) == tuple(fwd.args[:3]) and _sdpa_plain(u)]
+        if lse is None or len(bwds) != 1:
+            continue
+        bwd = bwds[0]
+        op_f, op_b = fwd.target, bwd.target
+        fwd.target, fwd.args = attn.sdpa_fwd, (op_f, *fwd.args)
+        bwd.target, bwd.args = attn.sdpa_bwd, (op_b, *bwd.args)
+        nf += 1
+        nb += 1
+        folded = _fold_qkv_cat(bwd)
+        if folded is None:
+            continue
+        cat, chain = folded
+        bwd.kwargs = {**bwd.kwargs, "fold_qkv": True}
+        with graph.inserting_after(bwd):
+            dqkv = graph.call_function(operator.getitem, (bwd, 3))
+        dqkv.meta["val"] = cat.meta.get("val")
+        cat.replace_all_uses_with(dqkv)
+        _erase_dead(graph, [cat] + chain)
+        ncat += 1
+    gm.recompile()
+    return nf, nb, ncat
+
+
 def dispatch_compute(gm, counts=None):
     from . import gemm, norm
     native_ln = os.environ.get("EDB_NATIVE_LN", "1") == "1"
@@ -1797,7 +1876,9 @@
     counts["swiglu"] = fuse_swiglu(gm) if os.environ.get("EDB_NATIVE_SWIGLU", "1") == "1" else (0, 0)
     counts["rope"] = fuse_rope(gm) if os.environ.get("EDB_NATIVE_ROPE", "1") == "1" else (0, 0)
     counts["clip"] = fuse_grad_clip(gm) if os.environ.get("EDB_NATIVE_CLIP", "1") == "1" else (0, 0)
+    counts["attn"] = fuse_attention(gm) if os.environ.get("EDB_NATIVE_ATTN", "1") == "1" else (0, 0, 0)
     n += sum(counts["rms_norm"]) + sum(counts["swiglu"]) + sum(counts["rope"]) + sum(counts["clip"])
+    n += sum(counts["attn"][:2])
     for node in gm.graph.nodes:
         if node.op != "call_function":
             continue
diff --git a/include/edb.h b/include/edb.h
--- a/include/edb.h
+++ b/include/edb.h
@@ -167,6 +167,15 @@
                       int accumulate, int idx_dtype, int dtype, void* stream);
 int edb_embedding_bwd_workspace(int64_t rows, int64_t V, size_t* bytes_out);
 
+int edb_attn_fwd(void* out, const int64_t* out_strides, float* lse, const void* q,
+                 const int64_t* q_strides, const void* k, const int64_t* k_strides, const void* v,
+                 const int64_t* v_strides, int B, int H, int T, void* stream);
+int edb_attn_bwd(void* dq, const int64_t* dq_strides, void* dk, const int64_t* dk_strides, void* dv,
+                 const int64_t* dv_strides, float* dsum, const void* dout,
+                 const int64_t* dout_strides, const void* q, const int64_t* q_strides, const void* k,
+                 const int64_t* k_strides, const void* v, const int64_t* v_strides, const void* out,
+                 const int64_t* out_strides, const float* lse, int B, int H, int T, void* stream);
+
 int edb_colsum(void* out, const void* x, void* workspace, int64_t rows, int64_t cols, int64_t ld,
                int dtype, void* stream);
 int edb_colsum_workspace(int64_t cols, size_t* bytes_out);
```

After: 346.3, median of 6. 1.4% higher.
